# MengAiDev/SmokePhysAI

Measured on AMD Instinct MI355X. Metric: simulated+encoded frames/sec at 256^2 grid, batch 64, higher is better.
Workload: dtype f32 stencil + bf16x3 encoder (split-bf16 MFMA, fp32 accumulate)

## Files before the change

smokephysai_amd/csrc/encoder.h:

```cpp
#pragma once
#include <mutex>
#include <vector>

#include "common.h"

namespace smk {

struct EncoderDev {
    float *w1;
    float *s1, *t1;
    float *w2t;
    float *s2, *t2;
    unsigned short *w1p;
    signed char *w2i;
    float *sw2;
    int *wsum;
    unsigned short *w2q;
    unsigned short *w2s;
};

struct EncoderSkip {
    std::mutex mu;
    float *table[3][3][2] = {};
    int *ws = nullptr;
    size_t ws_tiles = 0;
    std::vector<void *> retired;
    int64_t last_total = 0;
    const int *last_count = nullptr;
    void release();
};
hipError_t encoder_skip_stats(EncoderSkip &sk, int64_t *tiles_total, int64_t *tiles_run, hipStream_t st);

hipError_t launch_fold_weights(const smk_encoder_weights &w, const EncoderDev &e, hipStream_t st);
hipError_t launch_conv1_only(const float *frames, int64_t fstride, int B, int H, int W, const EncoderDev &e, float *act,
                             hipStream_t st);
hipError_t launch_encoder_f32(const float *frames, int64_t fstride, int B, int H, int W, const EncoderDev &e,
                              float *features, hipStream_t st);

hipError_t launch_encoder_bf16(const float *frames, int64_t fstride, int B, int H, int W, const EncoderDev &e,
                               float *features, bool x3, bool tokens, hipStream_t st, EncoderSkip *skip = nullptr);
hipError_t launch_encoder_b16(const float *frames, int64_t fstride, int B, int H, int W, const EncoderDev &e,
                              float *features, bool tokens, hipStream_t st, EncoderSkip *skip = nullptr);

hipError_t launch_encoder_i8(const float *frames, int64_t fstride, int B, int H, int W, const EncoderDev &e,
                             float *features, bool tokens, hipStream_t st, EncoderSkip *skip = nullptr);

size_t conv2_train_workspace_bytes();
hipError_t launch_conv2_train_dgrad(const float *dz, const float *weight, int B, int H, int W, float *dx, void *workspace, hipStream_t st);
size_t conv1_wgrad_workspace_bytes();
hipError_t launch_conv1_train_forward(const float *x, const float *weight, const float *bias, int B, int H, int W, float *z1, hipStream_t st);
hipError_t launch_conv1_train_wgrad(const float *dz, const float *x, int B, int H, int W, float *dw, float *db, void *workspace, hipStream_t st);
size_t conv2_wgrad_workspace_bytes(int nstreams);
int conv2_wgrad_streams();
hipError_t launch_conv2_train_wgrad(const float *dz, const float *a1, int B, int H, int W, float *dw, float *db, void *workspace, hipStream_t st);
hipError_t launch_conv2_train_forward(const float *a1, const float *weight, const float *bias, int B, int H, int W, float *z2, void *workspace,
                                      hipStream_t st);

}
```

smokephysai_amd/csrc/encoder.hip:

```cpp
#include "encoder.h"

#include <stdlib.h>

namespace smk {

typedef float f32x16 __attribute__((ext_vector_type(16)));

constexpr int ENC_TH = 8, ENC_TW = 32;
constexpr int ENC_AH = ENC_TH + 2, ENC_AW = ENC_TW + 2;
constexpr int ENC_XH = ENC_TH + 8, ENC_XW = ENC_TW + 8;
constexpr int ENC_ACS = ENC_AH * ENC_AW;

__global__ void k_fold_weights(smk_encoder_weights w, EncoderDev e) {
    int t = blockIdx.x * blockDim.x + threadIdx.x;
    if (t < 64) {
        float s = w.bn1_w[t] / sqrtf(w.bn1_var[t] + 1e-5f);
        e.s1[t] = s;
        e.t1[t] = (w.conv1_b[t] - w.bn1_mean[t]) * s + w.bn1_b[t];
    }
    if (t < 128) {
        float s = w.bn2_w[t] / sqrtf(w.bn2_var[t] + 1e-5f);
        e.s2[t] = s;
        e.t2[t] = (w.conv2_b[t] - w.bn2_mean[t]) * s + w.bn2_b[t];
    }
    if (t < 64 * 49) e.w1[t] = w.conv1_w[t];
    if (t < 9 * 64 * 128) {
        int o = t % 128, c = (t / 128) % 64, tap = t / (128 * 64);
        e.w2t[t] = w.conv2_w[((size_t)o * 64 + c) * 9 + tap];
    }
    __bf16 *w1p = reinterpret_cast<__bf16 *>(e.w1p), *w2q = reinterpret_cast<__bf16 *>(e.w2q);
    if (t < 64 * 64) {
        int c = t / 64, k = t % 64, ki = k >> 3, kj = k & 7;
        float v = (ki < 7 && kj < 7) ? w.conv1_w[c * 49 + ki * 7 + kj] : 0.f;
        __bf16 hi = (__bf16)v;
        w1p[t] = hi;
        w1p[64 * 64 + t] = (__bf16)(v - (float)hi);
    }
    if (t < 36 * 128 * 16) {
        int cc = t % 16, o = (t / 16) % 128, ks = t / (16 * 128);
        int tap = ks >> 2, c = (ks & 3) * 16 + cc;
        float v = w.conv2_w[((size_t)o * 64 + c) * 9 + tap];
        __bf16 hi = (__bf16)v;
        w2q[((size_t)(ks * 2 + 0) * 128 + o) * 16 + cc] = hi;
        w2q[((size_t)(ks * 2 + 1) * 128 + o) * 16 + cc] = (__bf16)(v - (float)hi);
        __bf16 *w2s = reinterpret_cast<__bf16 *>(e.w2s);
        const int ks2 = tap * 2 + (c >> 5), c32 = c & 31;
        w2s[((size_t)(ks2 * 2 + 0) * 128 + o) * 32 + c32] = hi;
        w2s[((size_t)(ks2 * 2 + 1) * 128 + o) * 32 + c32] = (__bf16)(v - (float)hi);
    }
}

__global__ __launch_bounds__(256) void k_quant_w2(smk_encoder_weights w, EncoderDev e) {
    __shared__ float red[256];
    __shared__ int sh_h, sh_l;
    const int o = blockIdx.x, tid = threadIdx.x;
    if (tid == 0) { sh_h = 0; sh_l = 0; }
    float m = 0.f;
    for (int k = tid; k < 576; k += 256) m = fmaxf(m, fabsf(w.conv2_w[(size_t)o * 576 + k]));
    red[tid] = m;
    __syncthreads();
    for (int sft = 128; sft > 0; sft >>= 1) {
        if (tid < sft) red[tid] = fmaxf(red[tid], red[tid + sft]);
        __syncthreads();
    }
    const float wmax = red[0];
    const float sw = wmax > 0.f ? wmax / 32512.0f : 1.0f;
    if (tid == 0) e.sw2[o] = sw;
    int sum_h = 0, sum_l = 0;
    for (int k = tid; k < 576; k += 256) {
        const int c = k / 9, tap = k - 9 * c;
        const int q = (int)rintf(w.conv2_w[(size_t)o * 576 + k] / sw);
        const int h = (q + 128) >> 8, l = q - (h << 8);
        const int ks = tap * 2 + (c >> 5), cc = c & 31;
        e.w2i[((size_t)(ks * 2 + 0) * 128 + o) * 32 + cc] = (signed char)h;
        e.w2i[((size_t)(ks * 2 + 1) * 128 + o) * 32 + cc] = (signed char)l;
        sum_h += h; sum_l += l;
    }
    atomicAdd(&sh_h, sum_h);
    atomicAdd(&sh_l, sum_l);
    __syncthreads();
    if (tid == 0) { e.wsum[o] = 128 * sh_h; e.wsum[128 + o] = 128 * sh_l; }
}

hipError_t launch_fold_weights(const smk_encoder_weights &w, const EncoderDev &e, hipStream_t st) {
    hipLaunchKernelGGL(k_quant_w2, dim3(128), dim3(256), 0, st, w, e);
    int n = 9 * 64 * 128;
    hipLaunchKernelGGL(k_fold_weights, dim3((n + 255) / 256), dim3(256), 0, st, w, e);
    return hipGetLastError();
}

template <int NC>
__device__ __forceinline__ void conv1_pixel(const float (&patch)[49], const float *__restrict__ w1,
                                            const float *__restrict__ s1, const float *__restrict__ t1, int c0,
                                            float (&out)[NC]) {
#pragma unroll
    for (int cc = 0; cc < NC; ++cc) {
        const float *wc = w1 + (c0 + cc) * 49;
        float acc = 0.f;
#pragma unroll
        for (int t = 0; t < 49; ++t) acc = fmaf(patch[t], wc[t], acc);
        float y = fmaf(acc, s1[c0 + cc], t1[c0 + cc]);
        out[cc] = y > 0.f ? y : 0.f;
    }
}

__global__ __launch_bounds__(256) void k_conv1_only(const float *frames, int64_t fstride, int H, int W, EncoderDev e, float *act) {
    int b = blockIdx.z;
    int j = blockIdx.x * 64 + threadIdx.x, i = blockIdx.y * 4 + threadIdx.y;
    if (i >= H || j >= W) return;
    const float *x = frames + (size_t)b * fstride;
    float patch[49];
#pragma unroll
    for (int ki = 0; ki < 7; ++ki)
#pragma unroll
        for (int kj = 0; kj < 7; ++kj) {
            int ii = i + ki - 3, jj = j + kj - 3;
            patch[ki * 7 + kj] = (ii >= 0 && ii < H && jj >= 0 && jj < W) ? x[(size_t)ii * W + jj] : 0.f;
        }
#pragma unroll 1
    for (int c0 = 0; c0 < 64; c0 += 4) {
        float o[4];
        conv1_pixel<4>(patch, e.w1, e.s1, e.t1, c0, o);
#pragma unroll
        for (int cc = 0; cc < 4; ++cc) act[(((size_t)b * 64 + c0 + cc) * H + i) * W + j] = o[cc];
    }
}

hipError_t launch_conv1_only(const float *frames, int64_t fstride, int B, int H, int W, const EncoderDev &e, float *act,
                             hipStream_t st) {
    dim3 grid(cdiv(W, 64), cdiv(H, 4), B), block(64, 4);
    hipLaunchKernelGGL(k_conv1_only, grid, block, 0, st, frames, fstride, H, W, e, act);
    return hipGetLastError();
}

constexpr int LDS_XS = ENC_XH * ENC_XW;
constexpr int LDS_A1 = 64 * ENC_ACS;
constexpr int LDS_W2 = 64 * 128;
constexpr int LDS_F32_TOTAL = LDS_XS + LDS_A1 + 2 * LDS_W2;
constexpr int A2_PITCH = 129;

template <int PS>
__global__ __launch_bounds__(512) void k_encoder_f32(const float *__restrict__ frames, int64_t fstride, int H, int W,
                                                     EncoderDev e, float *__restrict__ features) {
    extern __shared__ __attribute__((aligned(16))) float lds[];
    float *xs = lds, *a1s = lds + LDS_XS, *w2s = lds + LDS_XS + LDS_A1;
    const int tid = threadIdx.x, lane = tid & 63;
    const int wave = __builtin_amdgcn_readfirstlane(tid >> 6);
    const int b = blockIdx.z, r0 = blockIdx.y * ENC_TH, c0 = blockIdx.x * ENC_TW;
    const float *x = frames + (size_t)b * fstride;

    for (int k = tid; k < LDS_XS; k += 512) {
        int ii = r0 - 4 + k / ENC_XW, jj = c0 - 4 + k % ENC_XW;
        xs[k] = (ii >= 0 && ii < H && jj >= 0 && jj < W) ? x[(size_t)ii * W + jj] : 0.f;
    }
    float4 wreg[4];
    {
        const float4 *src = reinterpret_cast<const float4 *>(e.w2t);
#pragma unroll
        for (int q = 0; q < 4; ++q) wreg[q] = src[q * 512 + tid];
    }
    __syncthreads();

    for (int task = wave; task < 48; task += 8) {
        const int chunk = task % 6, cq = task / 6;
        const int pix = chunk * 64 + lane;
        if (pix < ENC_ACS) {
            const int ar = pix / ENC_AW, ac = pix % ENC_AW;
            const int ii = r0 - 1 + ar, jj = c0 - 1 + ac;
            float o[8];
            if (ii >= 0 && ii < H && jj >= 0 && jj < W) {
                float patch[49];
#pragma unroll
                for (int ki = 0; ki < 7; ++ki)
#pragma unroll
                    for (int kj = 0; kj < 7; ++kj) patch[ki * 7 + kj] = xs[(ar + ki) * ENC_XW + ac + kj];
                conv1_pixel<8>(patch, e.w1, e.s1, e.t1, cq * 8, o);
            } else {
#pragma unroll
                for (int cc = 0; cc < 8; ++cc) o[cc] = 0.f;
            }
#pragma unroll
            for (int cc = 0; cc < 8; ++cc) a1s[(cq * 8 + cc) * ENC_ACS + pix] = o[cc];
        }
    }
    {
        float4 *dst = reinterpret_cast<float4 *>(w2s);
#pragma unroll
        for (int q = 0; q < 4; ++q) dst[q * 512 + tid] = wreg[q];
    }
    __syncthreads();

    f32x16 acc[4];
#pragma unroll
    for (int n = 0; n < 4; ++n)
#pragma unroll
        for (int r = 0; r < 16; ++r) acc[n][r] = 0.f;
    const int l31 = lane & 31, hi = lane >> 5;
    for (int tap = 0; tap < 9; ++tap) {
        if (tap + 1 < 9) {
            const float4 *src = reinterpret_cast<const float4 *>(e.w2t + (size_t)(tap + 1) * LDS_W2);
#pragma unroll
            for (int q = 0; q < 4; ++q) wreg[q] = src[q * 512 + tid];
        }
        const int ki = tap / 3, kj = tap % 3;
        const float *ap = a1s + hi * ENC_ACS + (wave + ki) * ENC_AW + l31 + kj;
        const float *bp = w2s + (tap & 1) * LDS_W2 + hi * 128 + l31;
#pragma unroll 4
        for (int cp = 0; cp < 32; ++cp) {
            float a = ap[cp * 2 * ENC_ACS];
#pragma unroll
            for (int n = 0; n < 4; ++n) {
                float bv = bp[cp * 2 * 128 + n * 32];
                acc[n] = __builtin_amdgcn_mfma_f32_32x32x2f32(a, bv, acc[n], 0, 0, 0);
            }
        }
        if (tap + 1 < 9) {
            float4 *dst = reinterpret_cast<float4 *>(w2s + ((tap + 1) & 1) * LDS_W2);
#pragma unroll
            for (int q = 0; q < 4; ++q) dst[q * 512 + tid] = wreg[q];
        }
        __syncthreads();
    }

    float *a2s = lds;
#pragma unroll
    for (int n = 0; n < 4; ++n) {
        const int o = n * 32 + l31;
        const float s = e.s2[o], t = e.t2[o];
#pragma unroll
        for (int r = 0; r < 16; ++r) {
            const int col = (r & 3) + 8 * (r >> 2) + 4 * hi;
            float y = fmaf(acc[n][r], s, t);
            a2s[(wave * ENC_TW + col) * A2_PITCH + o] = y > 0.f ? y : 0.f;
        }
    }
    __syncthreads();
    constexpr int CELLS_R = ENC_TH / PS, CELLS_C = ENC_TW / PS;
    const int OW = 32, OHW = 32 * 32;
    for (int k = tid; k < CELLS_R * CELLS_C * 128; k += 512) {
        const int o = k & 127, cell = k >> 7, cr = cell / CELLS_C, cc = cell % CELLS_C;
        float sum = 0.f;
        for (int rr = 0; rr < PS; ++rr)
            for (int q = 0; q < PS; ++q) sum += a2s[((cr * PS + rr) * ENC_TW + cc * PS + q) * A2_PITCH + o];
        const int pi = r0 / PS + cr, pj = c0 / PS + cc;
        features[((size_t)b * 128 + o) * OHW + pi * OW + pj] = sum * (1.0f / (PS * PS));
    }
}

hipError_t launch_encoder_f32(const float *frames, int64_t fstride, int B, int H, int W, const EncoderDev &e,
                              float *features, hipStream_t st) {
    const int PS = H / 32;
    dim3 grid(W / ENC_TW, H / ENC_TH, B), block(512);
    size_t lds_bytes = sizeof(float) * (size_t)(LDS_F32_TOTAL > 256 * A2_PITCH ? LDS_F32_TOTAL : 256 * A2_PITCH);
    once_per_device((const void *)k_encoder_f32<8>, [&] {
        (void)hipFuncSetAttribute((const void *)k_encoder_f32<2>, hipFuncAttributeMaxDynamicSharedMemorySize, (int)lds_bytes);
        (void)hipFuncSetAttribute((const void *)k_encoder_f32<4>, hipFuncAttributeMaxDynamicSharedMemorySize, (int)lds_bytes);
        (void)hipFuncSetAttribute((const void *)k_encoder_f32<8>, hipFuncAttributeMaxDynamicSharedMemorySize, (int)lds_bytes);
    });
    switch (PS) {
        case 2: hipLaunchKernelGGL(k_encoder_f32<2>, grid, block, lds_bytes, st, frames, fstride, H, W, e, features); break;
        case 4: hipLaunchKernelGGL(k_encoder_f32<4>, grid, block, lds_bytes, st, frames, fstride, H, W, e, features); break;
        case 8: hipLaunchKernelGGL(k_encoder_f32<8>, grid, block, lds_bytes, st, frames, fstride, H, W, e, features); break;
        default: return hipErrorInvalidValue;
    }
    return hipGetLastError();
}

typedef __bf16 bf16x8 __attribute__((ext_vector_type(8)));
typedef __bf16 bf16x4 __attribute__((ext_vector_type(4)));

constexpr int B3_TH = 8, B3_TW = 16;
constexpr int B3_AW = B3_TW + 2, B3_APIX = (B3_TH + 2) * B3_AW;
constexpr int B3_XH = B3_TH + 9, B3_XW = B3_TW + 9;
constexpr int B3_XS_BYTES = ((B3_XH * B3_XW * 4 + 15) / 16) * 16;
constexpr int B3_A1_PITCH = 144;
constexpr int B3_A1_ROW = B3_AW * B3_A1_PITCH + 32;
constexpr int B3_A1_BYTES = (B3_TH + 2) * B3_A1_ROW;
template <bool X3> constexpr int b3_lds_bytes() { return B3_XS_BYTES + (X3 ? 2 : 1) * B3_A1_BYTES; }

__device__ __forceinline__ void split_bf16(float v, __bf16 &hi, __bf16 &lo) {
    hi = (__bf16)v;
    lo = (__bf16)(v - (float)hi);
}

template <bool X3>
__device__ __forceinline__ void mma3(f32x16 &acc, const bf16x8 &ah, const bf16x8 &al, const bf16x8 &bh, const bf16x8 &bl) {
    if (X3) {
        acc = __builtin_amdgcn_mfma_f32_32x32x16_bf16(al, bh, acc, 0, 0, 0);
        acc = __builtin_amdgcn_mfma_f32_32x32x16_bf16(ah, bl, acc, 0, 0, 0);
    }
    acc = __builtin_amdgcn_mfma_f32_32x32x16_bf16(ah, bh, acc, 0, 0, 0);
}

__device__ __forceinline__ float bn_relu(float a, float s, float t) {
    float y = fmaf(a, s, t);
    return y > 0.f ? y : 0.f;
}

constexpr int B3_W1_PITCH = 144;
constexpr int B3_W1_BYTES = 64 * B3_W1_PITCH;
constexpr int B3_ST_BYTES = 2 * 64 * 4;
template <bool X3> constexpr int b3_lds_total() { return b3_lds_bytes<X3>() + (X3 ? 2 : 1) * B3_W1_BYTES + B3_ST_BYTES; }

__device__ __forceinline__ int tiles_to_run(const int *__restrict__ list, const int *__restrict__ count, int ntiles) {
    return list ? __builtin_amdgcn_readfirstlane(*count) : ntiles;
}
__device__ __forceinline__ int tile_at(const int *__restrict__ list, int k) {
    return list ? __builtin_amdgcn_readfirstlane(list[k]) : k;
}

template <bool X3, int PS, bool TOKENS>
__global__ __launch_bounds__(256, 2) void k_encoder_bf16(const float *__restrict__ frames, int64_t fstride, int H, int W,
                                                      EncoderDev e, float *__restrict__ features, int lg_tiles_x,
                                                      int lg_tiles_per_frame, int ntiles, int stagger,
                                                      const int *__restrict__ list, const int *__restrict__ count) {
    extern __shared__ __attribute__((aligned(16))) unsigned char smem[];
    float *xs = reinterpret_cast<float *>(smem);
    unsigned char *a1h = smem + B3_XS_BYTES, *a1l = a1h + B3_A1_BYTES;
    unsigned char *w1s = a1h + (X3 ? 2 : 1) * B3_A1_BYTES;
    float *st1 = reinterpret_cast<float *>(w1s + (X3 ? 2 : 1) * B3_W1_BYTES);
    const int tid = threadIdx.x, lane = tid & 63, r = lane & 31, hi = lane >> 5;
    const int wave = __builtin_amdgcn_readfirstlane(tid >> 6);

    if (tid < 128) st1[tid] = tid < 64 ? e.s1[tid] : e.t1[tid - 64];
    {
        constexpr int NCH = (X3 ? 2 : 1) * 64 * 8;
        const uint4 *src = reinterpret_cast<const uint4 *>(e.w1p);
        for (int c = tid; c < NCH; c += 256) {
            const int row = c >> 3, u = c & 7;
            *reinterpret_cast<uint4 *>(w1s + row * B3_W1_PITCH + u * 16) = src[c];
        }
    }
    const int o = wave * 32 + r;
    const float s2 = e.s2[o], t2 = e.t2[o];
    const int lane_b = (o * 2 + hi) * 16;
    const __amdgpu_buffer_rsrc_t wrsrc =
        __builtin_amdgcn_make_buffer_rsrc(const_cast<unsigned short *>(e.w2q), 0, 36 * 2 * 4096, 0x00020000);
    typedef unsigned int u32x4 __attribute__((ext_vector_type(4)));
    auto load_b = [&](int kn, int part) -> uint4 {
        const u32x4 v = __builtin_amdgcn_raw_buffer_load_b128(wrsrc, lane_b, (kn * 2 + part) * 4096, 0);
        return make_uint4(v[0], v[1], v[2], v[3]);
    };
    constexpr int RING = 6;
    uint4 bqh[RING], bql[RING];
#pragma unroll
    for (int k = 0; k < RING - 1; ++k) {
        bqh[k] = load_b(k, 0);
        if (X3) bql[k] = load_b(k, 1);
    }
    const int lane_off = (r >> 4) * 4 * B3_A1_ROW + (r & 15) * B3_A1_PITCH + 8 * hi * 2;

    auto x_fetch = [&](int t, int k) -> float {
        if (k >= B3_XH * B3_XW) return 0.f;
        const int bb = t >> lg_tiles_per_frame, rem = t & ((1 << lg_tiles_per_frame) - 1);
        const int rr0 = (rem >> lg_tiles_x) * B3_TH, cc0 = (rem & ((1 << lg_tiles_x) - 1)) * B3_TW;
        const int row = k / B3_XW, col = k - row * B3_XW;
        const int ii = rr0 - 4 + row, jj = cc0 - 4 + col;
        const bool ok = row < B3_XH - 1 && col < B3_XW - 1 && ii >= 0 && ii < H && jj >= 0 && jj < W;
        return ok ? frames[(size_t)bb * fstride + (size_t)ii * W + jj] : 0.f;
    };
    int k = blockIdx.x;
    const int nrun = tiles_to_run(list, count, ntiles);
    if (nrun == ntiles) list = nullptr;
    int t = k < nrun ? tile_at(list, k) : 0;
    if (stagger > 0 && ((blockIdx.x / 256) & 1))
        for (int i = 0; i < stagger; ++i) __builtin_amdgcn_s_sleep(127);
    if (k < nrun) {
        xs[tid] = x_fetch(t, tid);
        if (tid + 256 < B3_XH * B3_XW) xs[tid + 256] = x_fetch(t, tid + 256);
    }
    __syncthreads();

    for (; k < nrun; k += gridDim.x) {
        const int b = t >> lg_tiles_per_frame, rem = t & ((1 << lg_tiles_per_frame) - 1);
        const int r0 = (rem >> lg_tiles_x) * B3_TH, c0 = (rem & ((1 << lg_tiles_x) - 1)) * B3_TW;

        __builtin_amdgcn_s_setprio(0);
        auto x_frags = [&](int pb, bf16x8 (&xh)[4], bf16x8 (&xl)[4], int &aoff, bool &valid, bool &inimg) {
            const int pix = pb * 32 + r;
            valid = pix < B3_APIX;
            const int pc = valid ? pix : B3_APIX - 1;
            const int ar = pc / B3_AW, ac = pc - ar * B3_AW;
            const int ii = r0 - 1 + ar, jj = c0 - 1 + ac;
            inimg = valid && ii >= 0 && ii < H && jj >= 0 && jj < W;
            aoff = ar * B3_A1_ROW + ac * B3_A1_PITCH;
            const float *xp = xs + (ar + hi) * B3_XW + ac;
#pragma unroll
            for (int s = 0; s < 4; ++s)
#pragma unroll
                for (int j = 0; j < 8; ++j) {
                    __bf16 vh, vl;
                    split_bf16(xp[s * 2 * B3_XW + j], vh, vl);
                    xh[s][j] = vh; xl[s][j] = vl;
                }
        };
        auto conv1_store = [&](const f32x16 &acc, int cb, int aoff, bool valid, bool inimg) {
#pragma unroll
            for (int q = 0; q < 4; ++q) {
                const int ch0 = cb * 32 + 8 * q + 4 * hi;
                const float4 sc = *reinterpret_cast<const float4 *>(st1 + ch0);
                const float4 sh = *reinterpret_cast<const float4 *>(st1 + 64 + ch0);
                const float scv[4] = {sc.x, sc.y, sc.z, sc.w}, shv[4] = {sh.x, sh.y, sh.z, sh.w};
                bf16x4 vh, vl;
#pragma unroll
                for (int i = 0; i < 4; ++i) {
                    const float y = inimg ? bn_relu(acc[4 * q + i], scv[i], shv[i]) : 0.f;
                    __bf16 a, bb;
                    split_bf16(y, a, bb);
                    vh[i] = a; vl[i] = bb;
                }
                if (valid) {
                    *reinterpret_cast<bf16x4 *>(a1h + aoff + ch0 * 2) = vh;
                    if (X3) *reinterpret_cast<bf16x4 *>(a1l + aoff + ch0 * 2) = vl;
                }
            }
        };
        {
            bf16x8 xh[4], xl[4];
            int aoff; bool valid, inimg;
            x_frags(wave, xh, xl, aoff, valid, inimg);
            f32x16 acc0, acc1;
#pragma unroll
            for (int g = 0; g < 16; ++g) { acc0[g] = 0.f; acc1[g] = 0.f; }
            const unsigned char *wrow = w1s + r * B3_W1_PITCH + 8 * hi * 2;
#pragma unroll
            for (int s = 0; s < 4; ++s) {
                const bf16x8 a0h = *reinterpret_cast<const bf16x8 *>(wrow + s * 32);
                const bf16x8 a1hh = *reinterpret_cast<const bf16x8 *>(wrow + 32 * B3_W1_PITCH + s * 32);
                const bf16x8 a0l = X3 ? *reinterpret_cast<const bf16x8 *>(wrow + B3_W1_BYTES + s * 32) : a0h;
                const bf16x8 a1l_ = X3 ? *reinterpret_cast<const bf16x8 *>(wrow + B3_W1_BYTES + 32 * B3_W1_PITCH + s * 32) : a1hh;
                mma3<X3>(acc0, a0h, a0l, xh[s], xl[s]);
                mma3<X3>(acc1, a1hh, a1l_, xh[s], xl[s]);
            }
            conv1_store(acc0, 0, aoff, valid, inimg);
            conv1_store(acc1, 1, aoff, valid, inimg);
        }
        {
            bf16x8 xh[4], xl[4];
            int aoff; bool valid, inimg;
            const int cb = wave & 1;
            x_frags(4 + (wave >> 1), xh, xl, aoff, valid, inimg);
            f32x16 acc;
#pragma unroll
            for (int g = 0; g < 16; ++g) acc[g] = 0.f;
            const unsigned char *wrow = w1s + (cb * 32 + r) * B3_W1_PITCH + 8 * hi * 2;
#pragma unroll
            for (int s = 0; s < 4; ++s) {
                const bf16x8 ah = *reinterpret_cast<const bf16x8 *>(wrow + s * 32);
                const bf16x8 al = X3 ? *reinterpret_cast<const bf16x8 *>(wrow + B3_W1_BYTES + s * 32) : ah;
                mma3<X3>(acc, ah, al, xh[s], xl[s]);
            }
            conv1_store(acc, cb, aoff, valid, inimg);
        }
        __syncthreads();
        __builtin_amdgcn_s_setprio(1);

        const int kn = k + gridDim.x;
        const int tn = kn < nrun ? tile_at(list, kn) : 0;
        float xr0 = 0.f, xr1 = 0.f;
        if (kn < nrun) {
            xr0 = x_fetch(tn, tid);
            xr1 = x_fetch(tn, tid + 256);
        }

        f32x16 acc[4];
#pragma unroll
        for (int mi = 0; mi < 4; ++mi)
#pragma unroll
            for (int g = 0; g < 16; ++g) acc[mi][g] = 0.f;
        auto load_a = [&](int k, bf16x8 (&ah)[4], bf16x8 (&al)[4]) {
            const int tap = k >> 2, ks = k & 3, ki = tap / 3, kj = tap - 3 * ki;
            const int abase = lane_off + ki * B3_A1_ROW + kj * B3_A1_PITCH + ks * 32;
#pragma unroll
            for (int mi = 0; mi < 4; ++mi) {
                ah[mi] = *reinterpret_cast<const bf16x8 *>(a1h + abase + mi * B3_A1_ROW);
                if (X3) al[mi] = *reinterpret_cast<const bf16x8 *>(a1l + abase + mi * B3_A1_ROW);
            }
        };
        bf16x8 ahA[4], alA[4], ahB[4], alB[4];
        load_a(0, ahA, alA);
        constexpr int UNR = 6;
#pragma unroll 1
        for (int k0 = 0; k0 < 36; k0 += UNR) {
#pragma unroll
            for (int u = 0; u < UNR; ++u) {
                const int k = k0 + u;
                {
                    int kn = k + RING - 1;
                    kn = kn >= 36 ? kn - 36 : kn;
                    kn = __builtin_amdgcn_readfirstlane(kn);
                    bqh[(u + RING - 1) % RING] = load_b(kn, 0);
                    if (X3) bql[(u + RING - 1) % RING] = load_b(kn, 1);
                }
                if (k + 1 < 36) {
                    if (u & 1) load_a(k + 1, ahA, alA); else load_a(k + 1, ahB, alB);
                }
                const bf16x8 bh = __builtin_bit_cast(bf16x8, bqh[u % RING]);
                const bf16x8 bl = X3 ? __builtin_bit_cast(bf16x8, bql[u % RING]) : bh;
#pragma unroll
                for (int mi = 0; mi < 4; ++mi) {
                    if (u & 1) mma3<X3>(acc[mi], ahB[mi], alB[mi], bh, bl); else mma3<X3>(acc[mi], ahA[mi], alA[mi], bh, bl);
                }
                constexpr int NMF = X3 ? 12 : 4, NDS = X3 ? 8 : 4, NVM = X3 ? 2 : 1;
#pragma unroll
                for (int i = 0; i < NMF; ++i) {
                    __builtin_amdgcn_sched_group_barrier(0x008, 1, 0);
                    if (i < NDS) __builtin_amdgcn_sched_group_barrier(0x100, 1, 0);
                    else if (i < NDS + NVM) __builtin_amdgcn_sched_group_barrier(0x020, 1, 0);
                }
                __builtin_amdgcn_sched_barrier(0);
            }
        }

        auto out_index = [&](int pi, int pj) -> size_t {
            return TOKENS ? ((size_t)b * 1024 + pi * 32 + pj) * 128 + o : ((size_t)b * 128 + o) * 1024 + pi * 32 + pj;
        };
        if (PS == 2) {
#pragma unroll
            for (int mp = 0; mp < 2; ++mp)
#pragma unroll
                for (int qr = 0; qr < 2; ++qr)
#pragma unroll
                    for (int qc = 0; qc < 2; ++qc)
#pragma unroll
                        for (int cg = 0; cg < 2; ++cg) {
                            float sum = 0.f;
#pragma unroll
                            for (int mi = 2 * mp; mi < 2 * mp + 2; ++mi)
#pragma unroll
                                for (int i = 2 * cg; i < 2 * cg + 2; ++i) sum += bn_relu(acc[mi][4 * (2 * qr + qc) + i], s2, t2);
                            features[out_index((r0 + 2 * mp + 4 * qr) / 2, (c0 + 8 * qc + 4 * hi + 2 * cg) / 2)] = sum * 0.25f;
                        }
        } else if (PS == 4) {
#pragma unroll
            for (int qr = 0; qr < 2; ++qr)
#pragma unroll
                for (int qc = 0; qc < 2; ++qc) {
                    float sum = 0.f;
#pragma unroll
                    for (int mi = 0; mi < 4; ++mi)
#pragma unroll
                        for (int i = 0; i < 4; ++i) sum += bn_relu(acc[mi][4 * (2 * qr + qc) + i], s2, t2);
                    features[out_index((r0 + 4 * qr) / 4, (c0 + 8 * qc + 4 * hi) / 4)] = sum * (1.0f / 16);
                }
        } else {
            float cell[2];
#pragma unroll
            for (int qc = 0; qc < 2; ++qc) {
                float sum = 0.f;
#pragma unroll
                for (int mi = 0; mi < 4; ++mi)
#pragma unroll
                    for (int qr = 0; qr < 2; ++qr)
#pragma unroll
                        for (int i = 0; i < 4; ++i) sum += bn_relu(acc[mi][4 * (2 * qr + qc) + i], s2, t2);
                cell[qc] = sum;
            }
            const float other0 = __shfl_xor(cell[0], 32), other1 = __shfl_xor(cell[1], 32);
            const float total = hi == 0 ? cell[0] + other0 : cell[1] + other1;
            features[out_index(r0 / 8, c0 / 8 + hi)] = total * (1.0f / 64);
        }

        xs[tid] = xr0;
        if (tid + 256 < B3_XH * B3_XW) xs[tid + 256] = xr1;
        __syncthreads();
        t = tn;
    }
}

#ifndef S16_PRIO_CONV1
#define S16_PRIO_CONV1 0
#define S16_PRIO_KLOOP 1
#endif
constexpr int S16_A1_BYTES = B3_APIX * 128;
constexpr int S16_LDS = B3_XS_BYTES + 2 * S16_A1_BYTES + 2 * B3_W1_BYTES + B3_ST_BYTES;
typedef float f32x4v __attribute__((ext_vector_type(4)));

template <int PS, bool TOKENS>
__global__ __launch_bounds__(256, 2) void k_encoder_b16(const float *__restrict__ frames, int64_t fstride, int H, int W,
                                                     EncoderDev e, float *__restrict__ features, int lg_tiles_x,
                                                     int lg_tiles_per_frame, int ntiles, int stagger,
                                                     const int *__restrict__ list, const int *__restrict__ count) {
    extern __shared__ __attribute__((aligned(16))) unsigned char smem[];
    unsigned int *xs = reinterpret_cast<unsigned int *>(smem);
    unsigned char *a1h = smem + B3_XS_BYTES, *a1l = a1h + S16_A1_BYTES;
    unsigned char *w1s = a1l + S16_A1_BYTES;
    float *st1 = reinterpret_cast<float *>(w1s + 2 * B3_W1_BYTES);
    const int tid = threadIdx.x, lane = tid & 63, r = lane & 31, hi = lane >> 5;
    const int wave = __builtin_amdgcn_readfirstlane(tid >> 6);

    if (tid < 128) st1[tid] = tid < 64 ? e.s1[tid] : e.t1[tid - 64];
    {
        const uint4 *src = reinterpret_cast<const uint4 *>(e.w1p);
        for (int c = tid; c < 2 * 64 * 8; c += 256) {
            const int row = c >> 3, u = c & 7;
            *reinterpret_cast<uint4 *>(w1s + row * B3_W1_PITCH + u * 16) = src[c];
        }
    }
    const int px = lane & 15, kg = lane >> 4;
    const int o0 = wave * 32 + px;
    const float s2a = e.s2[o0], t2a = e.t2[o0], s2b = e.s2[o0 + 16], t2b = e.t2[o0 + 16];
    const int lane_b = o0 * 64 + kg * 16;
    const __amdgpu_buffer_rsrc_t wrsrc =
        __builtin_amdgcn_make_buffer_rsrc(const_cast<unsigned short *>(e.w2s), 0, 18 * 2 * 8192, 0x00020000);
    typedef unsigned int u32x4 __attribute__((ext_vector_type(4)));
    auto load_b = [&](int ks, int part, int nt) -> uint4 {
        const u32x4 v = __builtin_amdgcn_raw_buffer_load_b128(wrsrc, lane_b, (ks * 2 + part) * 8192 + nt * 1024, 0);
        return make_uint4(v.x, v.y, v.z, v.w);
    };
    constexpr int RING = 2;
    uint4 bq[RING][2][2];
#pragma unroll
    for (int k = 0; k < RING - 1; ++k)
#pragma unroll
        for (int nt = 0; nt < 2; ++nt) {
            bq[k][nt][0] = load_b(k, 0, nt);
            bq[k][nt][1] = load_b(k, 1, nt);
        }

    auto x_fetch = [&](int t, int k) -> float {
        if (k >= B3_XH * B3_XW) return 0.f;
        const int bb = t >> lg_tiles_per_frame, rem = t & ((1 << lg_tiles_per_frame) - 1);
        const int rr0 = (rem >> lg_tiles_x) * B3_TH, cc0 = (rem & ((1 << lg_tiles_x) - 1)) * B3_TW;
        const int row = k / B3_XW, col = k - row * B3_XW;
        const int ii = rr0 - 4 + row, jj = cc0 - 4 + col;
        const bool ok = row < B3_XH - 1 && col < B3_XW - 1 && ii >= 0 && ii < H && jj >= 0 && jj < W;
        return ok ? frames[(size_t)bb * fstride + (size_t)ii * W + jj] : 0.f;
    };
    auto pack_split = [](float v) -> unsigned int {
        __bf16 vh, vl;
        split_bf16(v, vh, vl);
        return (unsigned int)__builtin_bit_cast(unsigned short, vh) | ((unsigned int)__builtin_bit_cast(unsigned short, vl) << 16);
    };
    int k = blockIdx.x;
    const int nrun = tiles_to_run(list, count, ntiles);
    if (nrun == ntiles) list = nullptr;
    int t = k < nrun ? tile_at(list, k) : 0;
    if (stagger > 0 && ((blockIdx.x / 256) & 1))
        for (int i = 0; i < stagger; ++i) __builtin_amdgcn_s_sleep(127);
    if (k < nrun) {
        xs[tid] = pack_split(x_fetch(t, tid));
        if (tid + 256 < B3_XH * B3_XW) xs[tid + 256] = pack_split(x_fetch(t, tid + 256));
    }
    __syncthreads();

    for (; k < nrun; k += gridDim.x) {
        const int b = t >> lg_tiles_per_frame, rem = t & ((1 << lg_tiles_per_frame) - 1);
        const int r0 = (rem >> lg_tiles_x) * B3_TH, c0 = (rem & ((1 << lg_tiles_x) - 1)) * B3_TW;

        __builtin_amdgcn_s_setprio(S16_PRIO_CONV1);
#ifdef SMK_ENC_ABLATE
        const bool abl_conv1 = !((SMK_ENC_ABLATE & 1) && k != (int)blockIdx.x);
#else
        constexpr bool abl_conv1 = true;
#endif
        auto x_frags = [&](int pb, bf16x8 (&xh)[4], bf16x8 (&xl)[4], int &pix, bool &valid, bool &inimg) {
            const int pp = pb * 32 + r;
            valid = pp < B3_APIX;
            pix = valid ? pp : B3_APIX - 1;
            const int ar = pix / B3_AW, ac = pix - ar * B3_AW;
            const int ii = r0 - 1 + ar, jj = c0 - 1 + ac;
            inimg = valid && ii >= 0 && ii < H && jj >= 0 && jj < W;
            const unsigned int *xp = xs + (ar + hi) * B3_XW + ac;
#pragma unroll
            for (int s = 0; s < 4; ++s) {
                unsigned int wh[4], wl[4];
#pragma unroll
                for (int jj = 0; jj < 4; ++jj) {
                    const unsigned int e0 = xp[s * 2 * B3_XW + 2 * jj], e1 = xp[s * 2 * B3_XW + 2 * jj + 1];
                    wh[jj] = __builtin_amdgcn_perm(e1, e0, 0x05040100u);
                    wl[jj] = __builtin_amdgcn_perm(e1, e0, 0x07060302u);
                }
                xh[s] = __builtin_bit_cast(bf16x8, make_uint4(wh[0], wh[1], wh[2], wh[3]));
                xl[s] = __builtin_bit_cast(bf16x8, make_uint4(wl[0], wl[1], wl[2], wl[3]));
            }
        };
        auto conv1_store = [&](const f32x16 &acc, int cb, int pix, bool valid, bool inimg) {
            const int sw = pix & 7;
#pragma unroll
            for (int q = 0; q < 4; ++q) {
                const int ch0 = cb * 32 + 8 * q + 4 * hi;
                const float4 sc = *reinterpret_cast<const float4 *>(st1 + ch0);
                const float4 sh = *reinterpret_cast<const float4 *>(st1 + 64 + ch0);
                const float scv[4] = {sc.x, sc.y, sc.z, sc.w}, shv[4] = {sh.x, sh.y, sh.z, sh.w};
                bf16x4 vh, vl;
#pragma unroll
                for (int i = 0; i < 4; ++i) {
                    const float y = inimg ? bn_relu(acc[4 * q + i], scv[i], shv[i]) : 0.f;
                    __bf16 a, bb;
                    split_bf16(y, a, bb);
                    vh[i] = a; vl[i] = bb;
                }
                if (valid) {
                    const int off = pix * 128 + (((cb * 4 + q) ^ sw) * 16) + 8 * hi;
                    *reinterpret_cast<bf16x4 *>(a1h + off) = vh;
                    *reinterpret_cast<bf16x4 *>(a1l + off) = vl;
                }
            }
        };
        if (abl_conv1) {
            bf16x8 xh[4], xl[4];
            int pix; bool valid, inimg;
            x_frags(wave, xh, xl, pix, valid, inimg);
            f32x16 acc0, acc1;
#pragma unroll
            for (int g = 0; g < 16; ++g) { acc0[g] = 0.f; acc1[g] = 0.f; }
            const unsigned char *wrow = w1s + r * B3_W1_PITCH + 8 * hi * 2;
#pragma unroll
            for (int s = 0; s < 4; ++s) {
                const bf16x8 a0h = *reinterpret_cast<const bf16x8 *>(wrow + s * 32);
                const bf16x8 a1hh = *reinterpret_cast<const bf16x8 *>(wrow + 32 * B3_W1_PITCH + s * 32);
                const bf16x8 a0l = *reinterpret_cast<const bf16x8 *>(wrow + B3_W1_BYTES + s * 32);
                const bf16x8 a1l_ = *reinterpret_cast<const bf16x8 *>(wrow + B3_W1_BYTES + 32 * B3_W1_PITCH + s * 32);
                mma3<true>(acc0, a0h, a0l, xh[s], xl[s]);
                mma3<true>(acc1, a1hh, a1l_, xh[s], xl[s]);
            }
            conv1_store(acc0, 0, pix, valid, inimg);
            conv1_store(acc1, 1, pix, valid, inimg);
        }
        if (abl_conv1) {
            bf16x8 xh[4], xl[4];
            int pix; bool valid, inimg;
            const int cb = wave & 1;
            x_frags(4 + (wave >> 1), xh, xl, pix, valid, inimg);
            f32x16 acc;
#pragma unroll
            for (int g = 0; g < 16; ++g) acc[g] = 0.f;
            const unsigned char *wrow = w1s + (cb * 32 + r) * B3_W1_PITCH + 8 * hi * 2;
#pragma unroll
            for (int s = 0; s < 4; ++s) {
                const bf16x8 ah = *reinterpret_cast<const bf16x8 *>(wrow + s * 32);
                const bf16x8 al = *reinterpret_cast<const bf16x8 *>(wrow + B3_W1_BYTES + s * 32);
                mma3<true>(acc, ah, al, xh[s], xl[s]);
            }
            conv1_store(acc, cb, pix, valid, inimg);
        }
#if !defined(SMK_ENC_ABLATE) || !(SMK_ENC_ABLATE & 4)
        __syncthreads();
#endif
        __builtin_amdgcn_s_setprio(S16_PRIO_KLOOP);

        const int kn = k + gridDim.x;
        const int tn = kn < nrun ? tile_at(list, kn) : 0;
        float xr0 = 0.f, xr1 = 0.f;
        if (kn < nrun) {
            xr0 = x_fetch(tn, tid);
            xr1 = x_fetch(tn, tid + 256);
        }

        f32x4v acc[8][2];
#pragma unroll
        for (int mt = 0; mt < 8; ++mt)
#pragma unroll
            for (int nt = 0; nt < 2; ++nt)
#pragma unroll
                for (int g = 0; g < 4; ++g) acc[mt][nt][g] = 0.f;
        const int c16[2] = {kg << 4, (4 + kg) << 4};
        auto tap_consts = [&](int ki, int kj, int (&om)[4]) {
#pragma unroll
            for (int m = 0; m < 4; ++m) om[m] = ((px + kj) << 7) ^ (((px + kj + 2 * (m + ki)) & 7) << 4);
        };
        auto load_a = [&](int ki, int half, int hm, const int (&om)[4], bf16x8 (&ah)[4], bf16x8 (&al)[4]) {
            const unsigned char *ph = a1h + ki * (B3_AW * 128), *pl = a1l + ki * (B3_AW * 128);
#pragma unroll
            for (int m = 0; m < 4; ++m) {
                const int off = om[m] ^ c16[half];
                ah[m] = *reinterpret_cast<const bf16x8 *>(ph + off + (4 * hm + m) * (B3_AW * 128));
                al[m] = *reinterpret_cast<const bf16x8 *>(pl + off + (4 * hm + m) * (B3_AW * 128));
            }
        };
        bf16x8 ahA[4], alA[4], ahB[4], alB[4];
        int om[4];
        tap_consts(0, 0, om);
        load_a(0, 0, 0, om, ahA, alA);
        int ki = 0, kj = 0;
#pragma unroll 1
        for (int tap = 0; tap < 9; ++tap) {
#pragma unroll
            for (int u = 0; u < 4; ++u) {
                const int half = u >> 1, hm = u & 1, slot = half % RING;
                if (hm == 0) {
                    int kn = tap * 2 + half + RING - 1;
                    kn = kn >= 18 ? kn - 18 : kn;
                    kn = __builtin_amdgcn_readfirstlane(kn);
#pragma unroll
                    for (int nt = 0; nt < 2; ++nt) {
                        bq[(slot + RING - 1) % RING][nt][0] = load_b(kn, 0, nt);
                        bq[(slot + RING - 1) % RING][nt][1] = load_b(kn, 1, nt);
                    }
                }
                if (u < 3) {
                    if (u & 1) load_a(ki, (u + 1) >> 1, (u + 1) & 1, om, ahA, alA);
                    else load_a(ki, (u + 1) >> 1, (u + 1) & 1, om, ahB, alB);
                } else if (tap < 8) {
                    kj = kj == 2 ? 0 : kj + 1;
                    ki = kj == 0 ? ki + 1 : ki;
                    tap_consts(ki, kj, om);
                    load_a(ki, 0, 0, om, ahA, alA);
                }
#pragma unroll
                for (int pr = 0; pr < 3; ++pr)
#pragma unroll
                    for (int m = 0; m < 4; ++m)
#pragma unroll
                        for (int nt = 0; nt < 2; ++nt) {
                            const bf16x8 bh = __builtin_bit_cast(bf16x8, bq[slot][nt][0]);
                            const bf16x8 bl = __builtin_bit_cast(bf16x8, bq[slot][nt][1]);
                            f32x4v &c = acc[4 * hm + m][nt];
                            const bf16x8 ah = (u & 1) ? ahB[m] : ahA[m], al = (u & 1) ? alB[m] : alA[m];
#if defined(SMK_ENC_ABLATE) && (SMK_ENC_ABLATE & 8)
                            asm volatile("" :: "v"(al), "v"(ah), "v"(bh), "v"(bl), "v"(c));
#else
                            if (pr == 0) c = __builtin_amdgcn_mfma_f32_16x16x32_bf16(al, bh, c, 0, 0, 0);
                            else if (pr == 1) c = __builtin_amdgcn_mfma_f32_16x16x32_bf16(ah, bl, c, 0, 0, 0);
                            else c = __builtin_amdgcn_mfma_f32_16x16x32_bf16(ah, bh, c, 0, 0, 0);
#endif
                        }
#pragma unroll
                for (int i = 0; i < 24; ++i) {
                    __builtin_amdgcn_sched_group_barrier(0x008, 1, 0);
                    if (i % 3 == 0) __builtin_amdgcn_sched_group_barrier(0x100, 1, 0);
                    else if (hm == 0 && (i == 1 || i == 2 || i == 4 || i == 5)) __builtin_amdgcn_sched_group_barrier(0x020, 1, 0);
                }
                __builtin_amdgcn_sched_barrier(0);
            }
        }

        auto out_index = [&](int pi, int pj, int o) -> size_t {
            return TOKENS ? ((size_t)b * 1024 + pi * 32 + pj) * 128 + o : ((size_t)b * 128 + o) * 1024 + pi * 32 + pj;
        };
#if defined(SMK_ENC_ABLATE) && (SMK_ENC_ABLATE & 2)
#pragma unroll
        for (int mt = 0; mt < 8; ++mt) asm volatile("" :: "v"(acc[mt][0]), "v"(acc[mt][1]));
        if (false)
#endif
#pragma unroll
        for (int nt = 0; nt < 2; ++nt) {
            const float s2 = nt ? s2b : s2a, t2 = nt ? t2b : t2a;
            const int o = o0 + 16 * nt;
            if (PS == 2) {
#pragma unroll
                for (int mp = 0; mp < 4; ++mp)
#pragma unroll
                    for (int cg = 0; cg < 2; ++cg) {
                        float sum = 0.f;
#pragma unroll
                        for (int mt = 2 * mp; mt < 2 * mp + 2; ++mt)
#pragma unroll
                            for (int i = 2 * cg; i < 2 * cg + 2; ++i) sum += bn_relu(acc[mt][nt][i], s2, t2);
                        features[out_index((r0 + 2 * mp) / 2, (c0 + 4 * kg + 2 * cg) / 2, o)] = sum * 0.25f;
                    }
            } else if (PS == 4) {
#pragma unroll
                for (int mq = 0; mq < 2; ++mq) {
                    float sum = 0.f;
#pragma unroll
                    for (int mt = 4 * mq; mt < 4 * mq + 4; ++mt)
#pragma unroll
                        for (int i = 0; i < 4; ++i) sum += bn_relu(acc[mt][nt][i], s2, t2);
                    features[out_index((r0 + 4 * mq) / 4, (c0 + 4 * kg) / 4, o)] = sum * (1.0f / 16);
                }
            } else {
                float sum = 0.f;
#pragma unroll
                for (int mt = 0; mt < 8; ++mt)
#pragma unroll
                    for (int i = 0; i < 4; ++i) sum += bn_relu(acc[mt][nt][i], s2, t2);
                const float other = __shfl_xor(sum, 16);
                const float total = (kg & 1) == 0 ? sum + other : other + sum;
                if ((kg & 1) == 0) features[out_index(r0 / 8, c0 / 8 + (kg >> 1), o)] = total * (1.0f / 64);
            }
        }

        xs[tid] = pack_split(xr0);
        if (tid + 256 < B3_XH * B3_XW) xs[tid + 256] = pack_split(xr1);
#if !defined(SMK_ENC_ABLATE) || !(SMK_ENC_ABLATE & 4)
        __syncthreads();
#endif
        t = tn;
    }
}

constexpr int C1_WP = 52;
__global__ __launch_bounds__(256) void k_conv1_train_fwd(const float *__restrict__ x, int H, int W, const float *__restrict__ w,
                                                        const float *__restrict__ bias, float *__restrict__ z1) {
    __shared__ __attribute__((aligned(16))) float ws[64 * C1_WP];
    __shared__ float xs[10][264];
    const int tid = threadIdx.x, b = blockIdx.z, i0 = blockIdx.y * 4, j0 = blockIdx.x * 256;
    for (int k = tid; k < 64 * C1_WP; k += 256) {
        const int c = k / C1_WP, t = k - c * C1_WP;
        ws[k] = t < 49 ? w[c * 49 + t] : 0.f;
    }
    const float *xb = x + (size_t)b * H * W;
    for (int k = tid; k < 10 * 262; k += 256) {
        const int r = k / 262, cc = k - r * 262, ii = i0 - 3 + r, jj = j0 - 3 + cc;
        const int ci = ii < 0 ? 0 : (ii > H - 1 ? H - 1 : ii), cj = jj < 0 ? 0 : (jj > W - 1 ? W - 1 : jj);
        const float v = xb[(size_t)ci * W + cj];
        xs[r][cc] = (ii == ci && jj == cj) ? v : 0.f;
    }
    __syncthreads();
    const int jq = tid & 63, row = tid >> 6;
    float win[7][10];
#pragma unroll
    for (int r = 0; r < 7; ++r)
#pragma unroll
        for (int cc = 0; cc < 10; ++cc) win[r][cc] = xs[row + r][4 * jq + cc];
    const int i = i0 + row, j = j0 + 4 * jq;
    if (i >= H || j >= W) return;
    float *dst = z1 + ((size_t)b * 64 * H + i) * W + j;
#pragma unroll 1
    for (int c = 0; c < 64; ++c) {
        float wv[C1_WP];
#pragma unroll
        for (int q = 0; q < C1_WP / 4; ++q) {
            const float4 t4 = *reinterpret_cast<const float4 *>(&ws[c * C1_WP + 4 * q]);
            wv[4 * q] = t4.x; wv[4 * q + 1] = t4.y; wv[4 * q + 2] = t4.z; wv[4 * q + 3] = t4.w;
        }
        float acc[4] = {0.f, 0.f, 0.f, 0.f};
#pragma unroll
        for (int ki = 0; ki < 7; ++ki)
#pragma unroll
            for (int kj = 0; kj < 7; ++kj)
#pragma unroll
                for (int p = 0; p < 4; ++p) acc[p] = fmaf(win[ki][kj + p], wv[ki * 7 + kj], acc[p]);
        const float bb = bias ? bias[c] : 0.f;
        *reinterpret_cast<float4 *>(dst + (size_t)c * H * W) = make_float4(acc[0] + bb, acc[1] + bb, acc[2] + bb, acc[3] + bb);
    }
}

constexpr int C1G_PX = 4 * 64;
constexpr int C1G_ZP = C1G_PX * 4 + 4;
__global__ __launch_bounds__(256) void k_conv1_train_wgrad(const float *__restrict__ dz, const float *__restrict__ x, int H, int W, int tiles_x,
                                                          int tiles_per_frame, int ntiles, float *__restrict__ part) {
    extern __shared__ __attribute__((aligned(16))) float smemf[];
    float *zs = smemf;
    float *xs = smemf + 16 * C1G_ZP;
    const int tid = threadIdx.x;
    const int st = tid / 112, rem = tid - st * 112, cg = rem / 7, ky = rem - cg * 7;
    float acc[4][7], dbs[4] = {0.f, 0.f, 0.f, 0.f};
#pragma unroll
    for (int c = 0; c < 4; ++c)
#pragma unroll
        for (int k = 0; k < 7; ++k) acc[c][k] = 0.f;
    const size_t plane = (size_t)H * W;
    for (int t = blockIdx.x; t < ntiles; t += gridDim.x) {
        const int b = t / tiles_per_frame, rm = t - b * tiles_per_frame;
        const int i0 = (rm / tiles_x) * 4, j0 = (rm % tiles_x) * 64;
#pragma unroll 4
        for (int k = 0; k < 16; ++k) {
            const int it = tid + 256 * k, g = it >> 8, p = it & 255, r = p >> 6, cc = p & 63;
            const float *src = dz + ((size_t)b * 64 + 4 * g) * plane + (size_t)(i0 + r) * W + j0 + cc;
            *reinterpret_cast<float4 *>(&zs[g * C1G_ZP + 4 * p]) = make_float4(src[0], src[plane], src[2 * plane], src[3 * plane]);
        }
        const float *xb = x + (size_t)b * plane;
        for (int k = tid; k < 10 * 70; k += 256) {
            const int r = k / 70, cc = k - r * 70, ii = i0 - 3 + r, jj = j0 - 3 + cc;
            const int ci = ii < 0 ? 0 : (ii > H - 1 ? H - 1 : ii), cj = jj < 0 ? 0 : (jj > W - 1 ? W - 1 : jj);
            const float v = xb[(size_t)ci * W + cj];
            xs[r * 72 + cc] = (ii == ci && jj == cj) ? v : 0.f;
        }
        __syncthreads();
        if (tid < 224) {
#pragma unroll 1
            for (int r = 2 * st; r < 2 * st + 2; ++r) {
                const float *xr = xs + (r + ky) * 72;
                float xv[7];
#pragma unroll
                for (int k = 0; k < 6; ++k) xv[k + 1] = xr[k];
#pragma unroll 4
                for (int cc = 0; cc < 64; ++cc) {
#pragma unroll
                    for (int k = 0; k < 6; ++k) xv[k] = xv[k + 1];
                    xv[6] = xr[cc + 6];
                    const float4 d = *reinterpret_cast<const float4 *>(&zs[cg * C1G_ZP + 4 * (r * 64 + cc)]);
                    const float dv[4] = {d.x, d.y, d.z, d.w};
#pragma unroll
                    for (int c = 0; c < 4; ++c) {
#pragma unroll
                        for (int k = 0; k < 7; ++k) acc[c][k] = fmaf(dv[c], xv[k], acc[c][k]);
                        if (ky == 0) dbs[c] += dv[c];
                    }
                }
            }
        }
        __syncthreads();
    }
    float *ex = smemf;
    if (st == 1 && tid < 224) {
#pragma unroll
        for (int c = 0; c < 4; ++c) {
#pragma unroll
            for (int k = 0; k < 7; ++k) ex[rem * 32 + c * 7 + k] = acc[c][k];
            ex[rem * 32 + 28 + c] = dbs[c];
        }
    }
    __syncthreads();
    if (st == 0) {
        float *dst = part + (size_t)blockIdx.x * (64 * 49 + 64);
#pragma unroll
        for (int c = 0; c < 4; ++c) {
#pragma unroll
            for (int k = 0; k < 7; ++k) dst[(4 * cg + c) * 49 + ky * 7 + k] = acc[c][k] + ex[rem * 32 + c * 7 + k];
            if (ky == 0) dst[64 * 49 + 4 * cg + c] = dbs[c] + ex[rem * 32 + 28 + c];
        }
    }
}

__global__ __launch_bounds__(256) void k_conv1_wgrad_finish(const float *__restrict__ part, int nparts, float *__restrict__ dw, float *__restrict__ db) {
    const int i = blockIdx.x * 256 + threadIdx.x;
    if (i >= 64 * 49 + 64) return;
    float s = 0.f;
    for (int k = 0; k < nparts; ++k) s += part[(size_t)k * (64 * 49 + 64) + i];
    if (i < 64 * 49) dw[i] = s;
    else if (db) db[i - 64 * 49] = s;
}

constexpr int C1G_LDS = (16 * C1G_ZP + 10 * 72) * 4;
int conv1_wgrad_parts() { return device_num_cu() * 2; }
size_t conv1_wgrad_workspace_bytes() { return (size_t)conv1_wgrad_parts() * (64 * 49 + 64) * sizeof(float); }

hipError_t launch_conv1_train_forward(const float *x, const float *weight, const float *bias, int B, int H, int W, float *z1, hipStream_t st) {
    if (W % 4 != 0 || B < 1) return hipErrorInvalidValue;
    hipLaunchKernelGGL(k_conv1_train_fwd, dim3(cdiv(W, 256), cdiv(H, 4), B), dim3(256), 0, st, x, H, W, weight, bias, z1);
    return hipGetLastError();
}

hipError_t launch_conv1_train_wgrad(const float *dz, const float *x, int B, int H, int W, float *dw, float *db, void *workspace, hipStream_t st) {
    if (H % 4 != 0 || W % 64 != 0 || B < 1) return hipErrorInvalidValue;
    const int tiles_x = W / 64, tiles_per_frame = tiles_x * (H / 4), ntiles = B * tiles_per_frame;
    int nparts = conv1_wgrad_parts();
    once_per_device((const void *)k_conv1_train_wgrad, [&] {
        (void)hipFuncSetAttribute((const void *)k_conv1_train_wgrad, hipFuncAttributeMaxDynamicSharedMemorySize, C1G_LDS);
    });
    const int grid = nparts < ntiles ? nparts : ntiles;
    float *part = static_cast<float *>(workspace);
    hipLaunchKernelGGL(k_conv1_train_wgrad, dim3(grid), dim3(256), C1G_LDS, st, dz, x, H, W, tiles_x, tiles_per_frame, ntiles, part);
    hipLaunchKernelGGL(k_conv1_wgrad_finish, dim3(cdiv(64 * 49 + 64, 256)), dim3(256), 0, st, part, grid, dw, db);
    return hipGetLastError();
}

constexpr int C2F_LDS = 3 * S16_A1_BYTES;
__device__ __forceinline__ void split3_bf16(float v, __bf16 &h, __bf16 &m, __bf16 &l) {
    h = (__bf16)v;
    const float r1 = v - (float)h;
    m = (__bf16)r1;
    l = (__bf16)(r1 - (float)m);
}

__global__ __launch_bounds__(256, 2) void k_conv2_fwd_b16(const float *__restrict__ a1, int H, int W, const unsigned short *__restrict__ w2s,
                                                       const float *__restrict__ bias, float *__restrict__ z2, int tiles_x,
                                                       int tiles_per_frame, int ntiles) {
    extern __shared__ __attribute__((aligned(16))) unsigned char smem[];
    unsigned char *a1p[3] = {smem, smem + S16_A1_BYTES, smem + 2 * S16_A1_BYTES};
    const int tid = threadIdx.x, lane = tid & 63;
    const int wave = __builtin_amdgcn_readfirstlane(tid >> 6);
    const int px = lane & 15, kg = lane >> 4;
    const int o0 = wave * 32 + px;
    const float b2a = bias ? bias[o0] : 0.f, b2b = bias ? bias[o0 + 16] : 0.f;
    const int lane_b = o0 * 64 + kg * 16;
    const __amdgpu_buffer_rsrc_t wrsrc =
        __builtin_amdgcn_make_buffer_rsrc(const_cast<unsigned short *>(w2s), 0, 18 * 3 * 8192, 0x00020000);
    typedef unsigned int u32x4 __attribute__((ext_vector_type(4)));
    auto load_b = [&](int ks, int part, int nt) -> uint4 {
        const u32x4 v = __builtin_amdgcn_raw_buffer_load_b128(wrsrc, lane_b, (ks * 3 + part) * 8192 + nt * 1024, 0);
        return make_uint4(v.x, v.y, v.z, v.w);
    };
    uint4 bq[2][2][3];
#pragma unroll
    for (int nt = 0; nt < 2; ++nt)
#pragma unroll
        for (int part = 0; part < 3; ++part) bq[0][nt][part] = load_b(0, part, nt);
    const size_t plane = (size_t)H * W;
    constexpr int ITEMS = (B3_TH + 2) * 8 * B3_AW;
    constexpr int NIT = (ITEMS + 255) / 256;

    for (int t = blockIdx.x; t < ntiles; t += gridDim.x) {
        const int b = t / tiles_per_frame, rem = t - b * tiles_per_frame;
        const int r0 = (rem / tiles_x) * B3_TH, c0 = (rem % tiles_x) * B3_TW;
        __builtin_amdgcn_s_setprio(S16_PRIO_CONV1);
        {
            const float *ab = a1 + (size_t)b * 64 * plane;
            float v[NIT][8];
#pragma unroll
            for (int j = 0; j < NIT; ++j) {
                int idx = tid + 256 * j;
                idx = idx < ITEMS ? idx : ITEMS - 1;
                const int row = idx / (8 * B3_AW), rm = idx - row * (8 * B3_AW), g = rm / B3_AW, pc = rm - g * B3_AW;
                const int ii = r0 - 1 + row, jj = c0 - 1 + pc;
                const int ci = ii < 0 ? 0 : (ii > H - 1 ? H - 1 : ii), cj = jj < 0 ? 0 : (jj > W - 1 ? W - 1 : jj);
                const float *src = ab + (size_t)(8 * g) * plane + (size_t)ci * W + cj;
#pragma unroll
                for (int c = 0; c < 8; ++c) v[j][c] = src[(size_t)c * plane];
            }
#pragma unroll
            for (int j = 0; j < NIT; ++j) {
                const int idx = tid + 256 * j;
                if (idx < ITEMS) {
                    const int row = idx / (8 * B3_AW), rm = idx - row * (8 * B3_AW), g = rm / B3_AW, pc = rm - g * B3_AW;
                    const int ii = r0 - 1 + row, jj = c0 - 1 + pc;
                    const bool in = ii >= 0 && ii < H && jj >= 0 && jj < W;
                    const int p = row * B3_AW + pc;
                    bf16x8 vh, vm, vl;
#pragma unroll
                    for (int c = 0; c < 8; ++c) {
                        __bf16 hh, mm, ll;
                        split3_bf16(in ? v[j][c] : 0.f, hh, mm, ll);
                        vh[c] = hh; vm[c] = mm; vl[c] = ll;
                    }
                    const int off = p * 128 + ((g ^ (p & 7)) * 16);
                    *reinterpret_cast<bf16x8 *>(a1p[0] + off) = vh;
                    *reinterpret_cast<bf16x8 *>(a1p[1] + off) = vm;
                    *reinterpret_cast<bf16x8 *>(a1p[2] + off) = vl;
                }
            }
        }
        __syncthreads();
        __builtin_amdgcn_s_setprio(S16_PRIO_KLOOP);

        f32x4v acc[8][2];
#pragma unroll
        for (int mt = 0; mt < 8; ++mt)
#pragma unroll
            for (int nt = 0; nt < 2; ++nt)
#pragma unroll
                for (int g = 0; g < 4; ++g) acc[mt][nt][g] = 0.f;
        const int c16[2] = {kg << 4, (4 + kg) << 4};
        auto tap_consts8 = [&](int ki, int kj, int (&om8)[8]) {
#pragma unroll
            for (int m = 0; m < 8; ++m) om8[m] = ((px + kj) << 7) ^ (((px + kj + 2 * (m + ki)) & 7) << 4);
        };
        auto load_a = [&](int ki, int half, int mq, const int (&om8)[8], bf16x8 (&af)[3][2]) {
#pragma unroll
            for (int j = 0; j < 2; ++j) {
                const int m = 2 * mq + j;
                const int off = (om8[m] ^ c16[half]) + (ki + m) * (B3_AW * 128);
#pragma unroll
                for (int part = 0; part < 3; ++part) af[part][j] = *reinterpret_cast<const bf16x8 *>(a1p[part] + off);
            }
        };
        bf16x8 afA[3][2], afB[3][2];
        int om8[8];
        tap_consts8(0, 0, om8);
        load_a(0, 0, 0, om8, afA);
        int ki = 0, kj = 0;
#pragma unroll 1
        for (int tap = 0; tap < 9; ++tap) {
#pragma unroll
            for (int u = 0; u < 8; ++u) {
                const int half = u >> 2, mq = u & 3, slot = half;
                if (mq == 0) {
                    int kn = tap * 2 + half + 1;
                    kn = kn >= 18 ? kn - 18 : kn;
                    kn = __builtin_amdgcn_readfirstlane(kn);
#pragma unroll
                    for (int nt = 0; nt < 2; ++nt)
#pragma unroll
                        for (int part = 0; part < 3; ++part) bq[slot ^ 1][nt][part] = load_b(kn, part, nt);
                }
                if (u < 7) {
                    if (u & 1) load_a(ki, (u + 1) >> 2, (u + 1) & 3, om8, afA);
                    else load_a(ki, (u + 1) >> 2, (u + 1) & 3, om8, afB);
                } else if (tap < 8) {
                    kj = kj == 2 ? 0 : kj + 1;
                    ki = kj == 0 ? ki + 1 : ki;
                    tap_consts8(ki, kj, om8);
                    load_a(ki, 0, 0, om8, afA);
                }
#pragma unroll
                for (int pr = 0; pr < 6; ++pr)
#pragma unroll
                    for (int j = 0; j < 2; ++j)
#pragma unroll
                        for (int nt = 0; nt < 2; ++nt) {
                            constexpr int PA[6] = {2, 0, 1, 1, 0, 0}, PB[6] = {0, 2, 1, 0, 1, 0};
                            const bf16x8 av = (u & 1) ? afB[PA[pr]][j] : afA[PA[pr]][j];
                            const bf16x8 bv = __builtin_bit_cast(bf16x8, bq[slot][nt][PB[pr]]);
                            f32x4v &c = acc[2 * mq + j][nt];
                            c = __builtin_amdgcn_mfma_f32_16x16x32_bf16(av, bv, c, 0, 0, 0);
                        }
#pragma unroll
                for (int i = 0; i < 24; ++i) {
                    __builtin_amdgcn_sched_group_barrier(0x008, 1, 0);
                    if (i % 4 == 0) __builtin_amdgcn_sched_group_barrier(0x100, 1, 0);
                    else if (mq == 0 && i < 9) __builtin_amdgcn_sched_group_barrier(0x020, 1, 0);
                }
                __builtin_amdgcn_sched_barrier(0);
            }
        }

#pragma unroll
        for (int nt = 0; nt < 2; ++nt) {
            const float bb = nt ? b2b : b2a;
            float *dst = z2 + ((size_t)b * 128 + o0 + 16 * nt) * plane + (size_t)r0 * W + c0 + 4 * kg;
#pragma unroll
            for (int mt = 0; mt < 8; ++mt) {
                const f32x4v c = acc[mt][nt];
                *reinterpret_cast<float4 *>(dst + (size_t)mt * W) = make_float4(c[0] + bb, c[1] + bb, c[2] + bb, c[3] + bb);
            }
        }
        __syncthreads();
    }
}

__global__ __launch_bounds__(256, 2) void k_conv2_dgrad_b16(const float *__restrict__ dz, int H, int W, const unsigned short *__restrict__ w2d,
                                                         float *__restrict__ dx, int tiles_x, int tiles_per_frame, int ntiles) {
    extern __shared__ __attribute__((aligned(16))) unsigned char smem[];
    unsigned char *a1h = smem, *a1l = a1h + S16_A1_BYTES;
    const int tid = threadIdx.x, lane = tid & 63;
    const int wave = __builtin_amdgcn_readfirstlane(tid >> 6);
    const int px = lane & 15, kg = lane >> 4;
    const int mh = wave & 1, nh = wave >> 1;
    const int c0o = nh * 32 + px;
    const int lane_b = c0o * 64 + kg * 16;
    const __amdgpu_buffer_rsrc_t wrsrc =
        __builtin_amdgcn_make_buffer_rsrc(const_cast<unsigned short *>(w2d), 0, 2 * 18 * 2 * 4096, 0x00020000);
    typedef unsigned int u32x4 __attribute__((ext_vector_type(4)));
    auto load_b = [&](int ks36, int part, int nt) -> uint4 {
        const u32x4 v = __builtin_amdgcn_raw_buffer_load_b128(wrsrc, lane_b, (ks36 * 2 + part) * 4096 + nt * 1024, 0);
        return make_uint4(v.x, v.y, v.z, v.w);
    };
    uint4 bq[2][2][2];
#pragma unroll
    for (int nt = 0; nt < 2; ++nt) {
        bq[0][nt][0] = load_b(0, 0, nt);
        bq[0][nt][1] = load_b(0, 1, nt);
    }
    const size_t plane = (size_t)H * W;
    constexpr int ITEMS = (B3_TH + 2) * 8 * B3_AW, NIT = (ITEMS + 255) / 256;
    const unsigned char *a1h_w = a1h + mh * 4 * (B3_AW * 128), *a1l_w = a1l + mh * 4 * (B3_AW * 128);
    const int c16[2] = {kg << 4, (4 + kg) << 4};

    for (int t = blockIdx.x; t < ntiles; t += gridDim.x) {
        const int b = t / tiles_per_frame, rem = t - b * tiles_per_frame;
        const int r0 = (rem / tiles_x) * B3_TH, c0 = (rem % tiles_x) * B3_TW;
        f32x4v acc[4][2];
#pragma unroll
        for (int m = 0; m < 4; ++m)
#pragma unroll
            for (int nt = 0; nt < 2; ++nt)
#pragma unroll
                for (int g = 0; g < 4; ++g) acc[m][nt][g] = 0.f;
#pragma unroll 1
        for (int pass = 0; pass < 2; ++pass) {
            __builtin_amdgcn_s_setprio(S16_PRIO_CONV1);
            {
                const float *ab = dz + ((size_t)b * 128 + 64 * pass) * plane;
                float v[NIT][8];
#pragma unroll
                for (int j = 0; j < NIT; ++j) {
                    int idx = tid + 256 * j;
                    idx = idx < ITEMS ? idx : ITEMS - 1;
                    const int row = idx / (8 * B3_AW), rm = idx - row * (8 * B3_AW), g = rm / B3_AW, pc = rm - g * B3_AW;
                    const int ii = r0 - 1 + row, jj = c0 - 1 + pc;
                    const int ci = ii < 0 ? 0 : (ii > H - 1 ? H - 1 : ii), cj = jj < 0 ? 0 : (jj > W - 1 ? W - 1 : jj);
                    const float *src = ab + (size_t)(8 * g) * plane + (size_t)ci * W + cj;
#pragma unroll
                    for (int c = 0; c < 8; ++c) v[j][c] = src[(size_t)c * plane];
                }
#pragma unroll
                for (int j = 0; j < NIT; ++j) {
                    const int idx = tid + 256 * j;
                    if (idx < ITEMS) {
                        const int row = idx / (8 * B3_AW), rm = idx - row * (8 * B3_AW), g = rm / B3_AW, pc = rm - g * B3_AW;
                        const int ii = r0 - 1 + row, jj = c0 - 1 + pc;
                        const bool in = ii >= 0 && ii < H && jj >= 0 && jj < W;
                        const int p = row * B3_AW + pc;
                        bf16x8 vh, vl;
#pragma unroll
                        for (int c = 0; c < 8; ++c) {
                            __bf16 hh, ll;
                            split_bf16(in ? v[j][c] : 0.f, hh, ll);
                            vh[c] = hh; vl[c] = ll;
                        }
                        const int off = p * 128 + ((g ^ (p & 7)) * 16);
                        *reinterpret_cast<bf16x8 *>(a1h + off) = vh;
                        *reinterpret_cast<bf16x8 *>(a1l + off) = vl;
                    }
                }
            }
            __syncthreads();
            __builtin_amdgcn_s_setprio(S16_PRIO_KLOOP);
            auto tap_consts = [&](int ki, int kj, int (&om)[4]) {
#pragma unroll
                for (int m = 0; m < 4; ++m) om[m] = ((px + kj) << 7) ^ (((px + kj + 2 * (m + ki)) & 7) << 4);
            };
            auto load_a = [&](int ki, int half, const int (&om)[4], bf16x8 (&ah)[4], bf16x8 (&al)[4]) {
                const unsigned char *ph = a1h_w + ki * (B3_AW * 128), *pl = a1l_w + ki * (B3_AW * 128);
#pragma unroll
                for (int m = 0; m < 4; ++m) {
                    const int off = om[m] ^ c16[half];
                    ah[m] = *reinterpret_cast<const bf16x8 *>(ph + off + m * (B3_AW * 128));
                    al[m] = *reinterpret_cast<const bf16x8 *>(pl + off + m * (B3_AW * 128));
                }
            };
            bf16x8 ahA[4], alA[4], ahB[4], alB[4];
            int om[4];
            tap_consts(0, 0, om);
            load_a(0, 0, om, ahA, alA);
            int ki = 0, kj = 0;
#pragma unroll 1
            for (int tap = 0; tap < 9; ++tap) {
#pragma unroll
                for (int half = 0; half < 2; ++half) {
                    const int slot = half;
                    {
                        int kn = pass * 18 + tap * 2 + half + 1;
                        kn = kn >= 36 ? kn - 36 : kn;
                        kn = __builtin_amdgcn_readfirstlane(kn);
#pragma unroll
                        for (int nt = 0; nt < 2; ++nt) {
                            bq[slot ^ 1][nt][0] = load_b(kn, 0, nt);
                            bq[slot ^ 1][nt][1] = load_b(kn, 1, nt);
                        }
                    }
                    if (half == 0) {
                        load_a(ki, 1, om, ahB, alB);
                    } else if (tap < 8) {
                        kj = kj == 2 ? 0 : kj + 1;
                        ki = kj == 0 ? ki + 1 : ki;
                        tap_consts(ki, kj, om);
                        load_a(ki, 0, om, ahA, alA);
                    }
#pragma unroll
                    for (int pr = 0; pr < 3; ++pr)
#pragma unroll
                        for (int m = 0; m < 4; ++m)
#pragma unroll
                            for (int nt = 0; nt < 2; ++nt) {
                                const bf16x8 bh = __builtin_bit_cast(bf16x8, bq[slot][nt][0]);
                                const bf16x8 bl = __builtin_bit_cast(bf16x8, bq[slot][nt][1]);
                                f32x4v &c = acc[m][nt];
                                const bf16x8 ah = half ? ahB[m] : ahA[m], al = half ? alB[m] : alA[m];
                                if (pr == 0) c = __builtin_amdgcn_mfma_f32_16x16x32_bf16(al, bh, c, 0, 0, 0);
                                else if (pr == 1) c = __builtin_amdgcn_mfma_f32_16x16x32_bf16(ah, bl, c, 0, 0, 0);
                                else c = __builtin_amdgcn_mfma_f32_16x16x32_bf16(ah, bh, c, 0, 0, 0);
                            }
#pragma unroll
                    for (int i = 0; i < 24; ++i) {
                        __builtin_amdgcn_sched_group_barrier(0x008, 1, 0);
                        if (i % 3 == 0) __builtin_amdgcn_sched_group_barrier(0x100, 1, 0);
                        else if (i == 1 || i == 2 || i == 4 || i == 5) __builtin_amdgcn_sched_group_barrier(0x020, 1, 0);
                    }
                    __builtin_amdgcn_sched_barrier(0);
                }
            }
            __syncthreads();
        }
#pragma unroll
        for (int nt = 0; nt < 2; ++nt) {
            float *dst = dx + ((size_t)b * 64 + c0o + 16 * nt) * plane + (size_t)(r0 + 4 * mh) * W + c0 + 4 * kg;
#pragma unroll
            for (int m = 0; m < 4; ++m) {
                const f32x4v c = acc[m][nt];
                *reinterpret_cast<float4 *>(dst + (size_t)m * W) = make_float4(c[0], c[1], c[2], c[3]);
            }
        }
    }
}

__global__ void k_split_conv2_weights_dgrad(const float *__restrict__ w, unsigned short *__restrict__ w2d_) {
    const int t = blockIdx.x * blockDim.x + threadIdx.x;
    if (t >= 9 * 64 * 128) return;
    const int o = t % 128, c = (t / 128) % 64, tap = t / (64 * 128);
    const float v = w[((size_t)o * 64 + c) * 9 + tap];
    const int ky = tap / 3, kx = tap - 3 * ky, tapf = (2 - ky) * 3 + (2 - kx);
    __bf16 *w2d = reinterpret_cast<__bf16 *>(w2d_);
    const __bf16 hi = (__bf16)v;
    const int pass = o >> 6, ol = o & 63, ks = tapf * 2 + (ol >> 5), o32 = ol & 31;
    const size_t base = ((size_t)(pass * 18 + ks) * 2) * 64 * 32;
    w2d[base + (size_t)c * 32 + o32] = hi;
    w2d[base + (size_t)64 * 32 + (size_t)c * 32 + o32] = (__bf16)(v - (float)hi);
}

hipError_t launch_conv2_train_dgrad(const float *dz, const float *weight, int B, int H, int W, float *dx, void *workspace, hipStream_t st) {
    if (H % B3_TH != 0 || W % B3_TW != 0 || B < 1) return hipErrorInvalidValue;
    unsigned short *w2d = static_cast<unsigned short *>(workspace);
    hipLaunchKernelGGL(k_split_conv2_weights_dgrad, dim3(cdiv(9 * 64 * 128, 256)), dim3(256), 0, st, weight, w2d);
    const int tiles_x = W / B3_TW, tiles_per_frame = tiles_x * (H / B3_TH), ntiles = B * tiles_per_frame;
    constexpr int lds = 2 * S16_A1_BYTES;
    const int wgs_per_cu = device_cached_int((const void *)k_conv2_dgrad_b16, [] {
        (void)hipFuncSetAttribute((const void *)k_conv2_dgrad_b16, hipFuncAttributeMaxDynamicSharedMemorySize, lds);
        int n = 0;
        if (hipOccupancyMaxActiveBlocksPerMultiprocessor(&n, (const void *)k_conv2_dgrad_b16, 256, lds) != hipSuccess || n < 1) n = 2;
        return n;
    });
    int nwg = device_num_cu() * wgs_per_cu;
    if (nwg > ntiles) nwg = ntiles;
    hipLaunchKernelGGL(k_conv2_dgrad_b16, dim3(nwg), dim3(256), lds, st, dz, H, W, w2d, dx, tiles_x, tiles_per_frame, ntiles);
    return hipGetLastError();
}

constexpr int WG_OG = 32;
constexpr int WG_ZP = 272;
constexpr int WG_AC = 336;
constexpr int WG_Z_BYTES = WG_OG * WG_ZP;
constexpr int WG_A_BYTES = 64 * WG_AC;
constexpr int WG_H_BYTES = 64 * 10 * 2 * 2;
constexpr int WG_LDS = 2 * (WG_Z_BYTES + WG_A_BYTES + WG_H_BYTES);

__global__ __launch_bounds__(256, 2) void k_conv2_wgrad_b16(const float *__restrict__ dz, const float *__restrict__ a1, int H, int W, int tiles_x,
                                                         int tiles_per_frame, int ntiles, int nstreams, float *__restrict__ part,
                                                         float *__restrict__ dbpart) {
    extern __shared__ __attribute__((aligned(16))) unsigned char smem[];
    unsigned char *zh = smem, *zl = zh + WG_Z_BYTES, *ah = zl + WG_Z_BYTES, *al = ah + WG_A_BYTES, *hh = al + WG_A_BYTES, *hl = hh + WG_H_BYTES;
    const int tid = threadIdx.x, lane = tid & 63;
    const int wave = __builtin_amdgcn_readfirstlane(tid >> 6);
    const int n15 = lane & 15, kg = lane >> 4;
    const int xcd = blockIdx.x & 7, og = (blockIdx.x >> 3) & 3, stream = (blockIdx.x >> 5) * 8 + xcd;
    const size_t plane = (size_t)H * W;
    f32x4v acc[2][9];
#pragma unroll
    for (int m = 0; m < 2; ++m)
#pragma unroll
        for (int t9 = 0; t9 < 9; ++t9)
#pragma unroll
            for (int g = 0; g < 4; ++g) acc[m][t9][g] = 0.f;
    float dbsum = 0.f;

    for (int t = stream; t < ntiles; t += nstreams) {
        const int b = t / tiles_per_frame, rem = t - b * tiles_per_frame;
        const int r0 = (rem / tiles_x) * B3_TH, c0 = (rem % tiles_x) * B3_TW;
        {
            const int o = tid >> 3, row = tid & 7;
            const float *src = dz + ((size_t)b * 128 + og * WG_OG + o) * plane + (size_t)(r0 + row) * W + c0;
            float4 v[4];
#pragma unroll
            for (int q = 0; q < 4; ++q) v[q] = *reinterpret_cast<const float4 *>(src + 4 * q);
#pragma unroll
            for (int hlf = 0; hlf < 2; ++hlf) {
                const float f[8] = {v[2 * hlf].x, v[2 * hlf].y, v[2 * hlf].z, v[2 * hlf].w, v[2 * hlf + 1].x, v[2 * hlf + 1].y, v[2 * hlf + 1].z, v[2 * hlf + 1].w};
                bf16x8 vh, vl;
#pragma unroll
                for (int c = 0; c < 8; ++c) {
                    __bf16 a_, b_;
                    split_bf16(f[c], a_, b_);
                    vh[c] = a_; vl[c] = b_;
                    dbsum += f[c];
                }
                const int off = o * WG_ZP + (row * 16 + 8 * hlf) * 2;
                *reinterpret_cast<bf16x8 *>(zh + off) = vh;
                *reinterpret_cast<bf16x8 *>(zl + off) = vl;
            }
        }
#pragma unroll
        for (int j = 0; j < 3; ++j) {
            const int it = tid + 256 * j;
            if (it < 640) {
                const int c = it / 10, row = it - c * 10;
                const int ii = r0 - 1 + row;
                const bool rin = ii >= 0 && ii < H;
                const float *src = a1 + ((size_t)b * 64 + c) * plane + (size_t)(rin ? ii : 0) * W + c0;
                float4 v[4];
#pragma unroll
                for (int q = 0; q < 4; ++q) v[q] = *reinterpret_cast<const float4 *>(src + 4 * q);
                const float lft = (rin && c0 > 0) ? src[-1] : 0.f, rgt = (rin && c0 + 16 < W) ? src[16] : 0.f;
#pragma unroll
                for (int hlf = 0; hlf < 2; ++hlf) {
                    const float f[8] = {v[2 * hlf].x, v[2 * hlf].y, v[2 * hlf].z, v[2 * hlf].w, v[2 * hlf + 1].x, v[2 * hlf + 1].y, v[2 * hlf + 1].z, v[2 * hlf + 1].w};
                    bf16x8 vh, vl;
#pragma unroll
                    for (int e = 0; e < 8; ++e) {
                        __bf16 a_, b_;
                        split_bf16(rin ? f[e] : 0.f, a_, b_);
                        vh[e] = a_; vl[e] = b_;
                    }
                    const int off = c * WG_AC + row * 32 + 16 * hlf;
                    *reinterpret_cast<bf16x8 *>(ah + off) = vh;
                    *reinterpret_cast<bf16x8 *>(al + off) = vl;
                }
                __bf16 lh_, ll_, rh_, rl_;
                split_bf16(lft, lh_, ll_);
                split_bf16(rgt, rh_, rl_);
                __bf16 *ph = reinterpret_cast<__bf16 *>(hh) + (c * 10 + row) * 2, *pl = reinterpret_cast<__bf16 *>(hl) + (c * 10 + row) * 2;
                ph[0] = lh_; ph[1] = rh_;
                pl[0] = ll_; pl[1] = rl_;
            }
        }
        __syncthreads();
        const int cw = wave * 16 + n15;
        const int x0 = 8 * (kg & 1);
#pragma unroll
        for (int s4 = 0; s4 < 4; ++s4) {
            const int prow = 2 * s4 + (kg >> 1);
            bf16x8 azh[2], azl[2];
#pragma unroll
            for (int m = 0; m < 2; ++m) {
                const int off = (m * 16 + n15) * WG_ZP + (prow * 16 + x0) * 2;
                azh[m] = *reinterpret_cast<const bf16x8 *>(zh + off);
                azl[m] = *reinterpret_cast<const bf16x8 *>(zl + off);
            }
#pragma unroll
            for (int ky = 0; ky < 3; ++ky) {
                const int arow = prow + ky;
                const int rbase = cw * WG_AC + arow * 32;
                typedef unsigned int u32x4 __attribute__((ext_vector_type(4)));
                const u32x4 ch = *reinterpret_cast<const u32x4 *>(ah + rbase + 2 * x0), cl = *reinterpret_cast<const u32x4 *>(al + rbase + 2 * x0);
                const int lo_off = x0 ? rbase + 14 : -1, ro_off = x0 ? -1 : rbase + 16;
                const int hidx = ((cw * 10 + arow) * 2) * 2;
                const unsigned int leh = lo_off >= 0 ? *reinterpret_cast<const unsigned short *>(ah + lo_off) : *reinterpret_cast<const unsigned short *>(hh + hidx);
                const unsigned int lel = lo_off >= 0 ? *reinterpret_cast<const unsigned short *>(al + lo_off) : *reinterpret_cast<const unsigned short *>(hl + hidx);
                const unsigned int reh = ro_off >= 0 ? *reinterpret_cast<const unsigned short *>(ah + ro_off) : *reinterpret_cast<const unsigned short *>(hh + hidx + 2);
                const unsigned int rel = ro_off >= 0 ? *reinterpret_cast<const unsigned short *>(al + ro_off) : *reinterpret_cast<const unsigned short *>(hl + hidx + 2);
#pragma unroll
                for (int kx = 0; kx < 3; ++kx) {
                    u32x4 fh, fl;
                    if (kx == 1) {
                        fh = ch; fl = cl;
                    } else if (kx == 0) {
                        fh[0] = leh | (ch[0] << 16); fl[0] = lel | (cl[0] << 16);
#pragma unroll
                        for (int i = 1; i < 4; ++i) {
                            fh[i] = __builtin_amdgcn_alignbit(ch[i], ch[i - 1], 16);
                            fl[i] = __builtin_amdgcn_alignbit(cl[i], cl[i - 1], 16);
                        }
                    } else {
#pragma unroll
                        for (int i = 0; i < 3; ++i) {
                            fh[i] = __builtin_amdgcn_alignbit(ch[i + 1], ch[i], 16);
                            fl[i] = __builtin_amdgcn_alignbit(cl[i + 1], cl[i], 16);
                        }
                        fh[3] = (ch[3] >> 16) | (reh << 16); fl[3] = (cl[3] >> 16) | (rel << 16);
                    }
                    const bf16x8 bh = __builtin_bit_cast(bf16x8, fh), bl = __builtin_bit_cast(bf16x8, fl);
                    const int t9 = ky * 3 + kx;
#pragma unroll
                    for (int m = 0; m < 2; ++m) {
                        f32x4v &c = acc[m][t9];
                        c = __builtin_amdgcn_mfma_f32_16x16x32_bf16(azl[m], bh, c, 0, 0, 0);
                        c = __builtin_amdgcn_mfma_f32_16x16x32_bf16(azh[m], bl, c, 0, 0, 0);
                        c = __builtin_amdgcn_mfma_f32_16x16x32_bf16(azh[m], bh, c, 0, 0, 0);
                    }
                }
            }
        }
        __syncthreads();
    }
    float *dst = part + ((size_t)stream * 4 + og) * (WG_OG * 9 * 64);
#pragma unroll
    for (int m = 0; m < 2; ++m)
#pragma unroll
        for (int t9 = 0; t9 < 9; ++t9)
#pragma unroll
            for (int g = 0; g < 4; ++g) dst[((size_t)(m * 16 + 4 * kg + g) * 9 + t9) * 64 + wave * 16 + n15] = acc[m][t9][g];
    float sdb = dbsum;
    sdb += __shfl_xor(sdb, 1); sdb += __shfl_xor(sdb, 2); sdb += __shfl_xor(sdb, 4);
    if ((tid & 7) == 0) dbpart[((size_t)stream * 4 + og) * WG_OG + (tid >> 3)] = sdb;
}

__global__ __launch_bounds__(256) void k_conv2_wgrad_finish(const float *__restrict__ part, const float *__restrict__ dbpart, int nstreams,
                                                          float *__restrict__ dw, float *__restrict__ db) {
    const int i = blockIdx.x * 256 + threadIdx.x;
    if (i < 128 * 9 * 64) {
        const int c = i & 63, t9 = (i >> 6) % 9, o = i / (9 * 64);
        const float *src = part + ((size_t)(o >> 5) * (WG_OG * 9 * 64)) + ((size_t)(o & 31) * 9 + t9) * 64 + c;
        float s = 0.f;
        for (int st = 0; st < nstreams; ++st) s += src[(size_t)st * 4 * (WG_OG * 9 * 64)];
        dw[((size_t)o * 64 + c) * 9 + t9] = s;
    }
    if (db && i < 128) {
        float s = 0.f;
        for (int st = 0; st < nstreams; ++st) s += dbpart[((size_t)st * 4 + (i >> 5)) * WG_OG + (i & 31)];
        db[i] = s;
    }
}

size_t conv2_wgrad_workspace_bytes(int nstreams) { return ((size_t)nstreams * 4 * (WG_OG * 9 * 64) + (size_t)nstreams * 4 * WG_OG) * sizeof(float); }
int conv2_wgrad_streams() { return (device_num_cu() * 2 / 32) * 8; }

hipError_t launch_conv2_train_wgrad(const float *dz, const float *a1, int B, int H, int W, float *dw, float *db, void *workspace, hipStream_t st) {
    if (H % B3_TH != 0 || W % B3_TW != 0 || B < 1) return hipErrorInvalidValue;
    const int tiles_x = W / B3_TW, tiles_per_frame = tiles_x * (H / B3_TH), ntiles = B * tiles_per_frame;
    const int nstreams = conv2_wgrad_streams();
    if (nstreams < 8) return hipErrorInvalidValue;
    float *part = static_cast<float *>(workspace), *dbpart = part + (size_t)nstreams * 4 * (WG_OG * 9 * 64);
    once_per_device((const void *)k_conv2_wgrad_b16, [&] {
        (void)hipFuncSetAttribute((const void *)k_conv2_wgrad_b16, hipFuncAttributeMaxDynamicSharedMemorySize, WG_LDS);
    });
    hipLaunchKernelGGL(k_conv2_wgrad_b16, dim3(nstreams * 4), dim3(256), WG_LDS, st, dz, a1, H, W, tiles_x, tiles_per_frame, ntiles, nstreams, part, dbpart);
    hipLaunchKernelGGL(k_conv2_wgrad_finish, dim3(cdiv(128 * 9 * 64, 256)), dim3(256), 0, st, part, dbpart, nstreams, dw, db);
    return hipGetLastError();
}

__global__ void k_split_conv2_weights(const float *__restrict__ w, unsigned short *__restrict__ w2s_) {
    const int t = blockIdx.x * blockDim.x + threadIdx.x;
    if (t >= 9 * 64 * 128) return;
    const int c = t % 64, o = (t / 64) % 128, tap = t / (64 * 128);
    const float v = w[((size_t)o * 64 + c) * 9 + tap];
    __bf16 *w2s = reinterpret_cast<__bf16 *>(w2s_);
    __bf16 h, m, l;
    split3_bf16(v, h, m, l);
    const int ks2 = tap * 2 + (c >> 5), c32 = c & 31;
    w2s[((size_t)(ks2 * 3 + 0) * 128 + o) * 32 + c32] = h;
    w2s[((size_t)(ks2 * 3 + 1) * 128 + o) * 32 + c32] = m;
    w2s[((size_t)(ks2 * 3 + 2) * 128 + o) * 32 + c32] = l;
}

size_t conv2_train_workspace_bytes() { return (size_t)18 * 3 * 128 * 32 * sizeof(unsigned short); }

hipError_t launch_conv2_train_forward(const float *a1, const float *weight, const float *bias, int B, int H, int W, float *z2, void *workspace,
                                      hipStream_t st) {
    if (H % B3_TH != 0 || W % B3_TW != 0 || B < 1) return hipErrorInvalidValue;
    unsigned short *w2s = static_cast<unsigned short *>(workspace);
    hipLaunchKernelGGL(k_split_conv2_weights, dim3(cdiv(9 * 64 * 128, 256)), dim3(256), 0, st, weight, w2s);
    const int tiles_x = W / B3_TW, tiles_per_frame = tiles_x * (H / B3_TH), ntiles = B * tiles_per_frame;
    constexpr int lds = C2F_LDS;
    const int wgs_per_cu = device_cached_int((const void *)k_conv2_fwd_b16, [] {
        (void)hipFuncSetAttribute((const void *)k_conv2_fwd_b16, hipFuncAttributeMaxDynamicSharedMemorySize, lds);
        int n = 0;
        if (hipOccupancyMaxActiveBlocksPerMultiprocessor(&n, (const void *)k_conv2_fwd_b16, 256, lds) != hipSuccess || n < 1) n = 2;
        return n;
    });
    int nwg = device_num_cu() * wgs_per_cu;
    if (nwg > ntiles) nwg = ntiles;
    hipLaunchKernelGGL(k_conv2_fwd_b16, dim3(nwg), dim3(256), lds, st, a1, H, W, w2s, bias, z2, tiles_x, tiles_per_frame, ntiles);
    return hipGetLastError();
}

struct EncoderKnobs {
    int stagger, wgs_per_cu, shape;
    bool skip;
    EncoderKnobs() {
        const char *sv = getenv("SMK_ENC_STAGGER"), *ov = getenv("SMK_ENC_WGS_PER_CU"), *sh = getenv("SMK_ENC_SHAPE");
        const char *sk = getenv("SMK_ENC_SKIP");
        stagger = sv ? atoi(sv) : 1;
        wgs_per_cu = ov && atoi(ov) > 0 ? atoi(ov) : 0;
        shape = sh && atoi(sh) == 32 ? 32 : 16;
        skip = !(sk && atoi(sk) == 0);
    }
};
static const EncoderKnobs &enc_knobs() {
    static const EncoderKnobs k;
    return k;
}

constexpr int SCAN_ROWS = 4;
constexpr int SCAN_BR = 2 * SCAN_ROWS + 2;
constexpr int SCAN_FW = 256 / 4 + 2;
constexpr int ENC_FRAME_FEATS = 128 * 1024;

template <int PS, bool TOKENS, bool VEC>
__global__ __launch_bounds__(256) void k_encoder_tile_scan(const float *__restrict__ frames, int64_t fstride, int H, int W, int lg_tiles_x,
                                                           int bands_per_frame, const float *__restrict__ table,
                                                           float *__restrict__ features, unsigned long long *__restrict__ masks) {
    __shared__ unsigned int flag[SCAN_BR][SCAN_FW];
    __shared__ unsigned long long s_mask;
    const int tid = threadIdx.x;
    const int band = blockIdx.x, b = band / bands_per_frame, bi = band - b * bands_per_frame;
    const int tiles_x = 1 << lg_tiles_x, band_tiles = SCAN_ROWS * tiles_x;
    for (int i = tid; i < SCAN_BR * SCAN_FW; i += 256) (&flag[0][0])[i] = 0;
    __syncthreads();
    const int W4 = W >> 2, row0 = bi * (SCAN_ROWS * B3_TH) - 4;
    const unsigned int *src = reinterpret_cast<const unsigned int *>(frames) + (size_t)b * fstride;
    for (int i = tid; i < SCAN_BR * 4 * W4; i += 256) {
        const int rr = i / W4, c4 = i - rr * W4, row = row0 + rr;
        if (row < 0 || row >= H) continue;
        const unsigned int *p = src + (size_t)row * W + 4 * c4;
        unsigned int any;
        if (VEC) {
            const uint4 v = *reinterpret_cast<const uint4 *>(p);
            any = v.x | v.y | v.z | v.w;
        } else {
            any = p[0] | p[1] | p[2] | p[3];
        }
        if (any) flag[rr >> 2][c4 + 1] = 1;
    }
    __syncthreads();
    if (tid < 64) {
        unsigned int any = 0;
        if (tid < band_tiles) {
            const int tyl = tid >> lg_tiles_x, tx = tid & (tiles_x - 1);
#pragma unroll
            for (int br = 0; br < 4; ++br)
#pragma unroll
                for (int bc = 0; bc < 6; ++bc) any |= flag[2 * tyl + br][4 * tx + bc];
        }
        const unsigned long long m = __ballot(any != 0);
        if (tid == 0) {
            s_mask = m;
            masks[band] = m;
        }
    }
    __syncthreads();
    const unsigned long long m = s_mask;
    constexpr int CR = B3_TH / PS, CC = B3_TW / PS;
    float *out = features + (size_t)b * ENC_FRAME_FEATS;
    const int ty0 = bi * SCAN_ROWS;
    if (TOKENS) {
        constexpr int ROWV = CC * 32, UPT = CR * ROWV;
        for (int i = tid; i < band_tiles * UPT; i += 256) {
            const int tl = i / UPT, u = i - tl * UPT;
            if ((m >> tl) & 1) continue;
            const int ty = ty0 + (tl >> lg_tiles_x), tx = tl & (tiles_x - 1);
            const int a = u / ROWV, q = u - a * ROWV;
            const size_t off = (size_t)((ty * CR + a) * 32 + tx * CC) * 128 + q * 4;
            *reinterpret_cast<float4 *>(out + off) = *reinterpret_cast<const float4 *>(table + off);
        }
    } else {
        constexpr int VW = CC < 4 ? CC : 4, VPR = CC / VW, UPT = 128 * CR * VPR;
        for (int i = tid; i < band_tiles * UPT; i += 256) {
            const int tl = i / UPT, u = i - tl * UPT;
            if ((m >> tl) & 1) continue;
            const int ty = ty0 + (tl >> lg_tiles_x), tx = tl & (tiles_x - 1);
            const int v = u % VPR, a = (u / VPR) % CR, o = u / (VPR * CR);
            const size_t off = (size_t)o * 1024 + (ty * CR + a) * 32 + tx * CC + v * VW;
            if (VW == 2) *reinterpret_cast<float2 *>(out + off) = *reinterpret_cast<const float2 *>(table + off);
            else *reinterpret_cast<float4 *>(out + off) = *reinterpret_cast<const float4 *>(table + off);
        }
    }
}

constexpr int PACK_BANDS = 4;
__global__ __launch_bounds__(64 * PACK_BANDS) void k_encoder_tile_scan_pack(const unsigned long long *__restrict__ masks, int nbands,
                                                                            int lg_band_tiles, int *__restrict__ list,
                                                                            int *__restrict__ count) {
    __shared__ int part[PACK_BANDS];
    const int tid = threadIdx.x, lane = tid & 63, wave = tid >> 6;
    const int first = blockIdx.x * PACK_BANDS, band = first + wave;
    int c = 0;
    for (int j = tid; j < first; j += 64 * PACK_BANDS) c += __popcll(masks[j]);
#pragma unroll
    for (int d = 32; d >= 1; d >>= 1) c += __shfl_xor(c, d);
    if (lane == 0) part[wave] = c;
    __syncthreads();
    int before = 0;
#pragma unroll
    for (int w = 0; w < PACK_BANDS; ++w) before += part[w];
    if (band >= nbands) return;
    for (int w = 0; w < wave; ++w) before += __popcll(masks[first + w]);
    const unsigned long long m = masks[band];
    if ((m >> lane) & 1) list[before + __popcll(m & ((1ull << lane) - 1))] = (band << lg_band_tiles) + lane;
    if (band == nbands - 1 && lane == 0) *count = before + __popcll(m);
}

void EncoderSkip::release() {
    for (auto &f : table)
        for (auto &h : f)
            for (float *&t : h) {
                if (t) (void)hipFree(t);
                t = nullptr;
            }
    if (ws) (void)hipFree(ws);
    for (void *p : retired) (void)hipFree(p);
    retired.clear();
    ws = nullptr;
    ws_tiles = 0;
    last_count = nullptr;
}

hipError_t encoder_skip_stats(EncoderSkip &sk, int64_t *tiles_total, int64_t *tiles_run, hipStream_t st) {
    std::lock_guard<std::mutex> lk(sk.mu);
    hipError_t err = hipStreamSynchronize(st);
    if (err != hipSuccess) return err;
    int n = 0;
    if (sk.last_count && (err = hipMemcpy(&n, sk.last_count, sizeof(int), hipMemcpyDeviceToHost)) != hipSuccess) return err;
    *tiles_total = sk.last_total;
    *tiles_run = sk.last_count ? n : sk.last_total;
    return hipSuccess;
}

struct SkipPlan {
    const int *list = nullptr, *count = nullptr;
};

template <int FORM, bool TOKENS, class ZeroLaunch>
static hipError_t skip_prepare(EncoderSkip *sk, const float *frames, int64_t fstride, int B, int H, int W, float *features, int lg_tx,
                               int ntiles, int nwg, hipStream_t st, ZeroLaunch zero_launch, SkipPlan &plan) {
    if (!sk) return hipSuccess;
    std::lock_guard<std::mutex> lk(sk->mu);
    sk->last_total = ntiles;
    sk->last_count = nullptr;
    if (!enc_knobs().skip || ntiles <= nwg || (reinterpret_cast<uintptr_t>(features) & 15)) return hipSuccess;
    hipStreamCaptureStatus cs = hipStreamCaptureStatusNone;
    if (hipStreamIsCapturing(st, &cs) != hipSuccess) {
        (void)hipGetLastError();
        return hipSuccess;
    }
    const bool capturing = cs != hipStreamCaptureStatusNone;
    hipError_t err;
    float *&tab = sk->table[FORM][H == 64 ? 0 : H == 128 ? 1 : 2][TOKENS ? 1 : 0];
    if (!tab) {
        if (capturing) return hipSuccess;
        float *p = nullptr;
        if ((err = hipMalloc((void **)&p, ((size_t)ENC_FRAME_FEATS + (size_t)H * W) * sizeof(float))) != hipSuccess) return err;
        err = hipMemsetAsync(p + ENC_FRAME_FEATS, 0, (size_t)H * W * sizeof(float), st);
        if (err == hipSuccess) err = zero_launch(p + ENC_FRAME_FEATS, p);
        if (err != hipSuccess) {
            (void)hipFree(p);
            return err;
        }
        tab = p;
    }
    if (sk->ws_tiles < (size_t)ntiles) {
        if (capturing) return hipSuccess;
        int *p = nullptr;
        if ((err = hipMalloc((void **)&p, (4 + (size_t)ntiles / 8 + (size_t)ntiles) * sizeof(int))) != hipSuccess) return err;
        if (sk->ws) sk->retired.push_back(sk->ws);
        sk->ws = p;
        sk->ws_tiles = ntiles;
    }
    int *count = sk->ws, *list = sk->ws + 4 + sk->ws_tiles / 8;
    unsigned long long *masks = reinterpret_cast<unsigned long long *>(sk->ws + 4);
    const int bands_per_frame = H / B3_TH / SCAN_ROWS, nbands = B * bands_per_frame;
    const bool vec = (reinterpret_cast<uintptr_t>(frames) & 15) == 0 && (fstride & 3) == 0;
    dim3 grid(nbands), block(256);
#define SMK_SCAN_LAUNCH(PS_, VEC_)                                                                                                  \
    hipLaunchKernelGGL((k_encoder_tile_scan<PS_, TOKENS, VEC_>), grid, block, 0, st, frames, fstride, H, W, lg_tx, bands_per_frame, \
                       (const float *)tab, features, masks)
    switch (H / 32) {
        case 2: if (vec) SMK_SCAN_LAUNCH(2, true); else SMK_SCAN_LAUNCH(2, false); break;
        case 4: if (vec) SMK_SCAN_LAUNCH(4, true); else SMK_SCAN_LAUNCH(4, false); break;
        case 8: if (vec) SMK_SCAN_LAUNCH(8, true); else SMK_SCAN_LAUNCH(8, false); break;
        default: return hipErrorInvalidValue;
    }
#undef SMK_SCAN_LAUNCH
    if ((err = hipGetLastError()) != hipSuccess) return err;
    hipLaunchKernelGGL(k_encoder_tile_scan_pack, dim3((nbands + PACK_BANDS - 1) / PACK_BANDS), dim3(64 * PACK_BANDS), 0, st,
                       (const unsigned long long *)masks, nbands, lg_tx + 2, list, count);
    if ((err = hipGetLastError()) != hipSuccess) return err;
    plan.list = list;
    plan.count = count;
    sk->last_count = count;
    return hipSuccess;
}

template <bool TOKENS>
static hipError_t launch_b16_t(const float *frames, int64_t fstride, int B, int H, int W, const EncoderDev &e, float *features,
                               hipStream_t st, EncoderSkip *skip) {
    const int PS = H / 32;
    const int tiles_x = W / B3_TW, tiles_per_frame = tiles_x * (H / B3_TH), ntiles = B * tiles_per_frame;
    int lg_tx = 0, lg_tpf = 0;
    while ((1 << lg_tx) < tiles_x) ++lg_tx;
    while ((1 << lg_tpf) < tiles_per_frame) ++lg_tpf;
    if ((1 << lg_tx) != tiles_x || (1 << lg_tpf) != tiles_per_frame || (PS != 2 && PS != 4 && PS != 8)) return hipErrorInvalidValue;
    const int stagger = enc_knobs().stagger;
    const int num_cu = device_num_cu();
    const int wgs_per_cu = device_cached_int((const void *)k_encoder_b16<8, TOKENS>, [] {
        (void)hipFuncSetAttribute((const void *)k_encoder_b16<8, TOKENS>, hipFuncAttributeMaxDynamicSharedMemorySize, S16_LDS);
        (void)hipFuncSetAttribute((const void *)k_encoder_b16<4, TOKENS>, hipFuncAttributeMaxDynamicSharedMemorySize, S16_LDS);
        (void)hipFuncSetAttribute((const void *)k_encoder_b16<2, TOKENS>, hipFuncAttributeMaxDynamicSharedMemorySize, S16_LDS);
        int n = 0;
        if (hipOccupancyMaxActiveBlocksPerMultiprocessor(&n, (const void *)k_encoder_b16<8, TOKENS>, 256, S16_LDS) != hipSuccess || n < 1) n = 2;
        return enc_knobs().wgs_per_cu ? enc_knobs().wgs_per_cu : n;
    });
    auto run = [&](const float *fr, int64_t fs, int nt, float *out, const int *list, const int *count) -> hipError_t {
        int nwg = num_cu * wgs_per_cu;
        if (nwg > nt) nwg = nt;
        dim3 grid(nwg), block(256);
        switch (PS) {
            case 2: hipLaunchKernelGGL((k_encoder_b16<2, TOKENS>), grid, block, S16_LDS, st, fr, fs, H, W, e, out, lg_tx, lg_tpf, nt, stagger, list, count); break;
            case 4: hipLaunchKernelGGL((k_encoder_b16<4, TOKENS>), grid, block, S16_LDS, st, fr, fs, H, W, e, out, lg_tx, lg_tpf, nt, stagger, list, count); break;
            default: hipLaunchKernelGGL((k_encoder_b16<8, TOKENS>), grid, block, S16_LDS, st, fr, fs, H, W, e, out, lg_tx, lg_tpf, nt, stagger, list, count); break;
        }
        return hipGetLastError();
    };
    SkipPlan plan;
    hipError_t err = skip_prepare<0, TOKENS>(
        skip, frames, fstride, B, H, W, features, lg_tx, ntiles, num_cu * wgs_per_cu, st,
        [&](const float *zero_frame, float *table) { return run(zero_frame, (int64_t)H * W, tiles_per_frame, table, nullptr, nullptr); },
        plan);
    if (err != hipSuccess) return err;
    return run(frames, fstride, ntiles, features, plan.list, plan.count);
}

hipError_t launch_encoder_b16(const float *frames, int64_t fstride, int B, int H, int W, const EncoderDev &e, float *features,
                              bool tokens, hipStream_t st, EncoderSkip *skip) {
    return tokens ? launch_b16_t<true>(frames, fstride, B, H, W, e, features, st, skip)
                  : launch_b16_t<false>(frames, fstride, B, H, W, e, features, st, skip);
}

template <bool X3, bool TOKENS>
static hipError_t launch_bf16_t(const float *frames, int64_t fstride, int B, int H, int W, const EncoderDev &e,
                                float *features, hipStream_t st, EncoderSkip *skip) {
    const int PS = H / 32;
    const int tiles_x = W / B3_TW, tiles_per_frame = tiles_x * (H / B3_TH), ntiles = tiles_per_frame * B;
    int lg_tx = 0, lg_tpf = 0;
    while ((1 << lg_tx) < tiles_x) ++lg_tx;
    while ((1 << lg_tpf) < tiles_per_frame) ++lg_tpf;
    if ((1 << lg_tx) != tiles_x || (1 << lg_tpf) != tiles_per_frame || (PS != 2 && PS != 4 && PS != 8)) return hipErrorInvalidValue;
    const int stagger = enc_knobs().stagger;
    constexpr size_t lds_bytes = b3_lds_total<X3>();
    const int num_cu = device_num_cu();
    const int wgs_per_cu = device_cached_int((const void *)k_encoder_bf16<X3, 8, TOKENS>, [] {
        constexpr size_t lb = b3_lds_total<X3>();
        (void)hipFuncSetAttribute((const void *)k_encoder_bf16<X3, 8, TOKENS>, hipFuncAttributeMaxDynamicSharedMemorySize, (int)lb);
        (void)hipFuncSetAttribute((const void *)k_encoder_bf16<X3, 4, TOKENS>, hipFuncAttributeMaxDynamicSharedMemorySize, (int)lb);
        (void)hipFuncSetAttribute((const void *)k_encoder_bf16<X3, 2, TOKENS>, hipFuncAttributeMaxDynamicSharedMemorySize, (int)lb);
        int n = 0;
        if (hipOccupancyMaxActiveBlocksPerMultiprocessor(&n, (const void *)k_encoder_bf16<X3, 8, TOKENS>, 256, lb) != hipSuccess || n < 1) n = 2;
        return enc_knobs().wgs_per_cu ? enc_knobs().wgs_per_cu : n;
    });
    auto run = [&](const float *fr, int64_t fs, int nt, float *out, const int *list, const int *count) -> hipError_t {
        int nwg = num_cu * wgs_per_cu;
        if (nwg > nt) nwg = nt;
        dim3 grid(nwg), block(256);
        switch (PS) {
            case 2: hipLaunchKernelGGL((k_encoder_bf16<X3, 2, TOKENS>), grid, block, lds_bytes, st, fr, fs, H, W, e, out, lg_tx, lg_tpf, nt, stagger, list, count); break;
            case 4: hipLaunchKernelGGL((k_encoder_bf16<X3, 4, TOKENS>), grid, block, lds_bytes, st, fr, fs, H, W, e, out, lg_tx, lg_tpf, nt, stagger, list, count); break;
            default: hipLaunchKernelGGL((k_encoder_bf16<X3, 8, TOKENS>), grid, block, lds_bytes, st, fr, fs, H, W, e, out, lg_tx, lg_tpf, nt, stagger, list, count); break;
        }
        return hipGetLastError();
    };
    SkipPlan plan;
    hipError_t err = skip_prepare<X3 ? 0 : 1, TOKENS>(
        skip, frames, fstride, B, H, W, features, lg_tx, ntiles, num_cu * wgs_per_cu, st,
        [&](const float *zero_frame, float *table) { return run(zero_frame, (int64_t)H * W, tiles_per_frame, table, nullptr, nullptr); },
        plan);
    if (err != hipSuccess) return err;
    return run(frames, fstride, ntiles, features, plan.list, plan.count);
}

hipError_t launch_encoder_bf16(const float *frames, int64_t fstride, int B, int H, int W, const EncoderDev &e,
                               float *features, bool x3, bool tokens, hipStream_t st, EncoderSkip *skip) {
    const int shape = enc_knobs().shape;
    if (x3 && shape == 16) return launch_encoder_b16(frames, fstride, B, H, W, e, features, tokens, st, skip);
    if (x3) return tokens ? launch_bf16_t<true, true>(frames, fstride, B, H, W, e, features, st, skip)
                          : launch_bf16_t<true, false>(frames, fstride, B, H, W, e, features, st, skip);
    return tokens ? launch_bf16_t<false, true>(frames, fstride, B, H, W, e, features, st, skip)
                  : launch_bf16_t<false, false>(frames, fstride, B, H, W, e, features, st, skip);
}

typedef int i32x16 __attribute__((ext_vector_type(16)));
typedef int i32x4 __attribute__((ext_vector_type(4)));

constexpr int I8_A1_PITCH = 80;
constexpr int I8_A1_ROW = B3_AW * I8_A1_PITCH + 32;
constexpr int I8_A1_BYTES = (B3_TH + 2) * I8_A1_ROW;
constexpr int I8_LDS_BYTES = B3_XS_BYTES + 2 * I8_A1_BYTES + 2 * B3_W1_BYTES + B3_ST_BYTES + 64;

template <int PS, bool TOKENS>
__global__ __launch_bounds__(256, 2) void k_encoder_i8(const float *__restrict__ frames, int64_t fstride, int H, int W,
                                                    EncoderDev e, float *__restrict__ features, int lg_tiles_x,
                                                    int lg_tiles_per_frame, int ntiles,
                                                    const int *__restrict__ list, const int *__restrict__ count) {
    extern __shared__ __attribute__((aligned(16))) unsigned char smem[];
    float *xs = reinterpret_cast<float *>(smem);
    unsigned char *a1h = smem + B3_XS_BYTES, *a1l = a1h + I8_A1_BYTES;
    unsigned char *w1s = a1l + I8_A1_BYTES;
    float *st1 = reinterpret_cast<float *>(w1s + 2 * B3_W1_BYTES);
    float *wmx = st1 + 128;
    const int tid = threadIdx.x, lane = tid & 63, r = lane & 31, hi = lane >> 5;
    const int wave = __builtin_amdgcn_readfirstlane(tid >> 6);

    if (tid < 128) st1[tid] = tid < 64 ? e.s1[tid] : e.t1[tid - 64];
    {
        const uint4 *src = reinterpret_cast<const uint4 *>(e.w1p);
        for (int c = tid; c < 2 * 64 * 8; c += 256) {
            const int row = c >> 3, u = c & 7;
            *reinterpret_cast<uint4 *>(w1s + row * B3_W1_PITCH + u * 16) = src[c];
        }
    }
    const int o = wave * 32 + r;
    const float t2 = e.t2[o];
    const float scale_o = e.sw2[o] * e.s2[o];
    const int corr_h = e.wsum[o], corr_l = e.wsum[128 + o];
    const int lane_b = (o * 2 + hi) * 16;
    const __amdgpu_buffer_rsrc_t wrsrc =
        __builtin_amdgcn_make_buffer_rsrc(const_cast<signed char *>(e.w2i), 0, 18 * 2 * 4096, 0x00020000);
    typedef unsigned int u32x4 __attribute__((ext_vector_type(4)));
    auto load_b = [&](int kn, int part) -> i32x4 {
        const u32x4 v = __builtin_amdgcn_raw_buffer_load_b128(wrsrc, lane_b, (kn * 2 + part) * 4096, 0);
        return __builtin_bit_cast(i32x4, v);
    };
    constexpr int RING = 3;
    i32x4 bqh[RING], bql[RING];
#pragma unroll
    for (int k = 0; k < RING - 1; ++k) {
        bqh[k] = load_b(k, 0);
        bql[k] = load_b(k, 1);
    }
    const int lane_off = (r >> 4) * 4 * I8_A1_ROW + (r & 15) * I8_A1_PITCH + 16 * hi;

    auto x_fetch = [&](int t, int k) -> float {
        if (k >= B3_XH * B3_XW) return 0.f;
        const int bb = t >> lg_tiles_per_frame, rem = t & ((1 << lg_tiles_per_frame) - 1);
        const int rr0 = (rem >> lg_tiles_x) * B3_TH, cc0 = (rem & ((1 << lg_tiles_x) - 1)) * B3_TW;
        const int row = k / B3_XW, col = k - row * B3_XW;
        const int ii = rr0 - 4 + row, jj = cc0 - 4 + col;
        const bool ok = row < B3_XH - 1 && col < B3_XW - 1 && ii >= 0 && ii < H && jj >= 0 && jj < W;
        return ok ? frames[(size_t)bb * fstride + (size_t)ii * W + jj] : 0.f;
    };
    int k = blockIdx.x;
    const int nrun = tiles_to_run(list, count, ntiles);
    if (nrun == ntiles) list = nullptr;
    int t = k < nrun ? tile_at(list, k) : 0;
    if (k < nrun) {
        xs[tid] = x_fetch(t, tid);
        if (tid + 256 < B3_XH * B3_XW) xs[tid + 256] = x_fetch(t, tid + 256);
    }
    __syncthreads();

    for (; k < nrun; k += gridDim.x) {
        const int b = t >> lg_tiles_per_frame, rem = t & ((1 << lg_tiles_per_frame) - 1);
        const int r0 = (rem >> lg_tiles_x) * B3_TH, c0 = (rem & ((1 << lg_tiles_x) - 1)) * B3_TW;

        __builtin_amdgcn_s_setprio(0);
        float yv[3][16];
        int aoffs[2];
        bool valids[2];
        float vmax = 0.f;
        auto x_frags = [&](int pb, bf16x8 (&xh)[4], bf16x8 (&xl)[4], int &aoff, bool &valid, bool &inimg) {
            const int pix = pb * 32 + r;
            valid = pix < B3_APIX;
            const int pc = valid ? pix : B3_APIX - 1;
            const int ar = pc / B3_AW, ac = pc - ar * B3_AW;
            const int ii = r0 - 1 + ar, jj = c0 - 1 + ac;
            inimg = valid && ii >= 0 && ii < H && jj >= 0 && jj < W;
            aoff = ar * I8_A1_ROW + ac * I8_A1_PITCH;
            const float *xp = xs + (ar + hi) * B3_XW + ac;
#pragma unroll
            for (int s = 0; s < 4; ++s)
#pragma unroll
                for (int j = 0; j < 8; ++j) {
                    __bf16 vh, vl;
                    split_bf16(xp[s * 2 * B3_XW + j], vh, vl);
                    xh[s][j] = vh; xl[s][j] = vl;
                }
        };
        bool inimgs[2];
        auto bn1 = [&](const f32x16 &acc, int cb, bool inimg, float (&y)[16]) {
            float umax = 0.f;
#pragma unroll
            for (int q = 0; q < 4; ++q) {
                const int ch0 = cb * 32 + 8 * q + 4 * hi;
                const float4 sc = *reinterpret_cast<const float4 *>(st1 + ch0);
                const float4 sh = *reinterpret_cast<const float4 *>(st1 + 64 + ch0);
                const float scv[4] = {sc.x, sc.y, sc.z, sc.w}, shv[4] = {sh.x, sh.y, sh.z, sh.w};
#pragma unroll
                for (int i = 0; i < 4; ++i) {
                    const float v = bn_relu(acc[4 * q + i], scv[i], shv[i]);
                    y[4 * q + i] = v;
                    umax = fmaxf(umax, v);
                }
            }
            vmax = fmaxf(vmax, inimg ? umax : 0.f);
        };
        {
            bf16x8 xh[4], xl[4];
            bool inimg;
            x_frags(wave, xh, xl, aoffs[0], valids[0], inimg);
            inimgs[0] = inimg;
            f32x16 acc0, acc1;
#pragma unroll
            for (int g = 0; g < 16; ++g) { acc0[g] = 0.f; acc1[g] = 0.f; }
            const unsigned char *wrow = w1s + r * B3_W1_PITCH + 8 * hi * 2;
#pragma unroll
            for (int s = 0; s < 4; ++s) {
                const bf16x8 a0h = *reinterpret_cast<const bf16x8 *>(wrow + s * 32);
                const bf16x8 a1hh = *reinterpret_cast<const bf16x8 *>(wrow + 32 * B3_W1_PITCH + s * 32);
                const bf16x8 a0l = *reinterpret_cast<const bf16x8 *>(wrow + B3_W1_BYTES + s * 32);
                const bf16x8 a1l_ = *reinterpret_cast<const bf16x8 *>(wrow + B3_W1_BYTES + 32 * B3_W1_PITCH + s * 32);
                mma3<true>(acc0, a0h, a0l, xh[s], xl[s]);
                mma3<true>(acc1, a1hh, a1l_, xh[s], xl[s]);
            }
            bn1(acc0, 0, inimg, yv[0]);
            bn1(acc1, 1, inimg, yv[1]);
        }
        const int cbs = wave & 1;
        {
            bf16x8 xh[4], xl[4];
            bool inimg;
            x_frags(4 + (wave >> 1), xh, xl, aoffs[1], valids[1], inimg);
            inimgs[1] = inimg;
            f32x16 acc;
#pragma unroll
            for (int g = 0; g < 16; ++g) acc[g] = 0.f;
            const unsigned char *wrow = w1s + (cbs * 32 + r) * B3_W1_PITCH + 8 * hi * 2;
#pragma unroll
            for (int s = 0; s < 4; ++s) {
                const bf16x8 ah = *reinterpret_cast<const bf16x8 *>(wrow + s * 32);
                const bf16x8 al = *reinterpret_cast<const bf16x8 *>(wrow + B3_W1_BYTES + s * 32);
                mma3<true>(acc, ah, al, xh[s], xl[s]);
            }
            bn1(acc, cbs, inimg, yv[2]);
        }
#pragma unroll
        for (int off = 32; off > 0; off >>= 1) vmax = fmaxf(vmax, __shfl_xor(vmax, off));
        if (lane == 0) wmx[wave] = vmax;
        __syncthreads();
        const float tmax = fmaxf(fmaxf(wmx[0], wmx[1]), fmaxf(wmx[2], wmx[3]));
        const float invn = tmax > 0.f ? 65024.0f / (tmax * 65535.0f) : 0.f;
        const float s_tile = tmax > 0.f ? tmax / 65024.0f : 0.f;
        constexpr float OFFN = 128.0f / 65535.0f;
        auto quant_store = [&](const float (&y)[16], int cb, int aoff, bool valid, bool inimg) {
            if (!valid) return;
#pragma unroll
            for (int q = 0; q < 4; ++q) {
                const int ch0 = cb * 32 + 8 * q + 4 * hi;
                const unsigned int d0 = __builtin_bit_cast(unsigned int, __builtin_amdgcn_cvt_pknorm_u16(
                    fmaf(y[4 * q + 0], invn, OFFN), fmaf(y[4 * q + 1], invn, OFFN)));
                const unsigned int d1 = __builtin_bit_cast(unsigned int, __builtin_amdgcn_cvt_pknorm_u16(
                    fmaf(y[4 * q + 2], invn, OFFN), fmaf(y[4 * q + 3], invn, OFFN)));
                unsigned int ph = __builtin_amdgcn_perm(d1, d0, 0x07050301) ^ 0x80808080u;
                unsigned int pl = __builtin_amdgcn_perm(d1, d0, 0x06040200) ^ 0x80808080u;
                ph = inimg ? ph : 0x80808080u;
                pl = inimg ? pl : 0u;
                *reinterpret_cast<unsigned int *>(a1h + aoff + ch0) = ph;
                *reinterpret_cast<unsigned int *>(a1l + aoff + ch0) = pl;
            }
        };
        quant_store(yv[0], 0, aoffs[0], valids[0], inimgs[0]);
        quant_store(yv[1], 1, aoffs[0], valids[0], inimgs[0]);
        quant_store(yv[2], cbs, aoffs[1], valids[1], inimgs[1]);
        __syncthreads();
        __builtin_amdgcn_s_setprio(1);

        const int kn = k + gridDim.x;
        const int tn = kn < nrun ? tile_at(list, kn) : 0;
        float xr0 = 0.f, xr1 = 0.f;
        if (kn < nrun) {
            xr0 = x_fetch(tn, tid);
            xr1 = x_fetch(tn, tid + 256);
        }

        i32x16 hh[4], mid[4];
#pragma unroll
        for (int mi = 0; mi < 4; ++mi)
#pragma unroll
            for (int g = 0; g < 16; ++g) { hh[mi][g] = corr_h; mid[mi][g] = corr_l; }
        auto load_a = [&](int k, int pair, i32x4 (&ah)[2], i32x4 (&al)[2]) {
            const int tap = k >> 1, half = k & 1, ki = tap / 3, kj = tap - 3 * ki;
            const int abase = lane_off + ki * I8_A1_ROW + kj * I8_A1_PITCH + half * 32 + pair * 2 * I8_A1_ROW;
#pragma unroll
            for (int m = 0; m < 2; ++m) {
                ah[m] = *reinterpret_cast<const i32x4 *>(a1h + abase + m * I8_A1_ROW);
                al[m] = *reinterpret_cast<const i32x4 *>(a1l + abase + m * I8_A1_ROW);
            }
        };
        i32x4 ahA[2], alA[2], ahB[2], alB[2];
        load_a(0, 0, ahA, alA);
#pragma unroll 1
        for (int k0 = 0; k0 < 18; k0 += 6) {
#pragma unroll
            for (int u = 0; u < 6; ++u) {
                const int k = k0 + u;
                {
                    int kn = k + RING - 1;
                    kn = kn >= 18 ? kn - 18 : kn;
                    kn = __builtin_amdgcn_readfirstlane(kn);
                    bqh[(u + RING - 1) % RING] = load_b(kn, 0);
                    bql[(u + RING - 1) % RING] = load_b(kn, 1);
                }
                const i32x4 bh = bqh[u % RING], bl = bql[u % RING];
                load_a(k, 1, ahB, alB);
#pragma unroll
                for (int m = 0; m < 2; ++m) {
                    mid[m] = __builtin_amdgcn_mfma_i32_32x32x32_i8(alA[m], bh, mid[m], 0, 0, 0);
                    mid[m] = __builtin_amdgcn_mfma_i32_32x32x32_i8(ahA[m], bl, mid[m], 0, 0, 0);
                    hh[m] = __builtin_amdgcn_mfma_i32_32x32x32_i8(ahA[m], bh, hh[m], 0, 0, 0);
                }
#pragma unroll
                for (int i = 0; i < 6; ++i) {
                    __builtin_amdgcn_sched_group_barrier(0x008, 1, 0);
                    if (i < 4) __builtin_amdgcn_sched_group_barrier(0x100, 1, 0);
                    else __builtin_amdgcn_sched_group_barrier(0x020, 1, 0);
                }
                __builtin_amdgcn_sched_barrier(0);
                if (k + 1 < 18) load_a(k + 1, 0, ahA, alA);
#pragma unroll
                for (int m = 0; m < 2; ++m) {
                    mid[2 + m] = __builtin_amdgcn_mfma_i32_32x32x32_i8(alB[m], bh, mid[2 + m], 0, 0, 0);
                    mid[2 + m] = __builtin_amdgcn_mfma_i32_32x32x32_i8(ahB[m], bl, mid[2 + m], 0, 0, 0);
                    hh[2 + m] = __builtin_amdgcn_mfma_i32_32x32x32_i8(ahB[m], bh, hh[2 + m], 0, 0, 0);
                }
#pragma unroll
                for (int i = 0; i < 6; ++i) {
                    __builtin_amdgcn_sched_group_barrier(0x008, 1, 0);
                    if (i < 4) __builtin_amdgcn_sched_group_barrier(0x100, 1, 0);
                }
                __builtin_amdgcn_sched_barrier(0);
            }
        }

        const float sc = s_tile * scale_o * 256.0f;
        auto val = [&](int mi, int g) -> float {
            const float v = fmaf((float)hh[mi][g], 256.0f, (float)mid[mi][g]);
            const float y = fmaf(v, sc, t2);
            return y > 0.f ? y : 0.f;
        };
        auto out_index = [&](int pi, int pj) -> size_t {
            return TOKENS ? ((size_t)b * 1024 + pi * 32 + pj) * 128 + o : ((size_t)b * 128 + o) * 1024 + pi * 32 + pj;
        };
        if (PS == 2) {
#pragma unroll
            for (int mp = 0; mp < 2; ++mp)
#pragma unroll
                for (int qr = 0; qr < 2; ++qr)
#pragma unroll
                    for (int qc = 0; qc < 2; ++qc)
#pragma unroll
                        for (int cg = 0; cg < 2; ++cg) {
                            float sum = 0.f;
#pragma unroll
                            for (int mi = 2 * mp; mi < 2 * mp + 2; ++mi)
#pragma unroll
                                for (int i = 2 * cg; i < 2 * cg + 2; ++i) sum += val(mi, 4 * (2 * qr + qc) + i);
                            features[out_index((r0 + 2 * mp + 4 * qr) / 2, (c0 + 8 * qc + 4 * hi + 2 * cg) / 2)] = sum * 0.25f;
                        }
        } else if (PS == 4) {
#pragma unroll
            for (int qr = 0; qr < 2; ++qr)
#pragma unroll
                for (int qc = 0; qc < 2; ++qc) {
                    float sum = 0.f;
#pragma unroll
                    for (int mi = 0; mi < 4; ++mi)
#pragma unroll
                        for (int i = 0; i < 4; ++i) sum += val(mi, 4 * (2 * qr + qc) + i);
                    features[out_index((r0 + 4 * qr) / 4, (c0 + 8 * qc + 4 * hi) / 4)] = sum * (1.0f / 16);
                }
        } else {
            float cell[2];
#pragma unroll
            for (int qc = 0; qc < 2; ++qc) {
                float sum = 0.f;
#pragma unroll
                for (int mi = 0; mi < 4; ++mi)
#pragma unroll
                    for (int qr = 0; qr < 2; ++qr)
#pragma unroll
                        for (int i = 0; i < 4; ++i) sum += val(mi, 4 * (2 * qr + qc) + i);
                cell[qc] = sum;
            }
            const float other0 = __shfl_xor(cell[0], 32), other1 = __shfl_xor(cell[1], 32);
            const float total = hi == 0 ? cell[0] + other0 : cell[1] + other1;
            features[out_index(r0 / 8, c0 / 8 + hi)] = total * (1.0f / 64);
        }

        xs[tid] = xr0;
        if (tid + 256 < B3_XH * B3_XW) xs[tid + 256] = xr1;
        __syncthreads();
        t = tn;
    }
}

template <bool TOKENS>
static hipError_t launch_i8_t(const float *frames, int64_t fstride, int B, int H, int W, const EncoderDev &e, float *features,
                              hipStream_t st, EncoderSkip *skip) {
    const int PS = H / 32;
    const int tiles_x = W / B3_TW, tiles_per_frame = tiles_x * (H / B3_TH), ntiles = tiles_per_frame * B;
    int lg_tx = 0, lg_tpf = 0;
    while ((1 << lg_tx) < tiles_x) ++lg_tx;
    while ((1 << lg_tpf) < tiles_per_frame) ++lg_tpf;
    if ((1 << lg_tx) != tiles_x || (1 << lg_tpf) != tiles_per_frame || (PS != 2 && PS != 4 && PS != 8)) return hipErrorInvalidValue;
    constexpr size_t lds_bytes = I8_LDS_BYTES;
    const int num_cu = device_num_cu();
    const int wgs_per_cu = device_cached_int((const void *)k_encoder_i8<8, TOKENS>, [] {
        int n = 0;
        if (hipOccupancyMaxActiveBlocksPerMultiprocessor(&n, (const void *)k_encoder_i8<8, TOKENS>, 256, I8_LDS_BYTES) != hipSuccess || n < 1) n = 2;
        return enc_knobs().wgs_per_cu ? enc_knobs().wgs_per_cu : n;
    });
    auto run = [&](const float *fr, int64_t fs, int nt, float *out, const int *list, const int *count) -> hipError_t {
        int nwg = num_cu * wgs_per_cu;
        if (nwg > nt) nwg = nt;
        dim3 grid(nwg), block(256);
        switch (PS) {
            case 2: hipLaunchKernelGGL((k_encoder_i8<2, TOKENS>), grid, block, lds_bytes, st, fr, fs, H, W, e, out, lg_tx, lg_tpf, nt, list, count); break;
            case 4: hipLaunchKernelGGL((k_encoder_i8<4, TOKENS>), grid, block, lds_bytes, st, fr, fs, H, W, e, out, lg_tx, lg_tpf, nt, list, count); break;
            default: hipLaunchKernelGGL((k_encoder_i8<8, TOKENS>), grid, block, lds_bytes, st, fr, fs, H, W, e, out, lg_tx, lg_tpf, nt, list, count); break;
        }
        return hipGetLastError();
    };
    SkipPlan plan;
    hipError_t err = skip_prepare<2, TOKENS>(
        skip, frames, fstride, B, H, W, features, lg_tx, ntiles, num_cu * wgs_per_cu, st,
        [&](const float *zero_frame, float *table) { return run(zero_frame, (int64_t)H * W, tiles_per_frame, table, nullptr, nullptr); },
        plan);
    if (err != hipSuccess) return err;
    return run(frames, fstride, ntiles, features, plan.list, plan.count);
}

hipError_t launch_encoder_i8(const float *frames, int64_t fstride, int B, int H, int W, const EncoderDev &e, float *features,
                             bool tokens, hipStream_t st, EncoderSkip *skip) {
    return tokens ? launch_i8_t<true>(frames, fstride, B, H, W, e, features, st, skip)
                  : launch_i8_t<false>(frames, fstride, B, H, W, e, features, st, skip);
}

}
```

Before: 216,900.

## Fuse skip-list compaction and zero-tile fill into encoder kernels

```diff
diff --git a/smokephysai_amd/csrc/encoder.h b/smokephysai_amd/csrc/encoder.h
--- a/smokephysai_amd/csrc/encoder.h
+++ b/smokephysai_amd/csrc/encoder.h
@@ -23,7 +23,7 @@
     std::mutex mu;
     float *table[3][3][2] = {};
     int *ws = nullptr;
-    size_t ws_tiles = 0;
+    size_t ws_bands = 0;
     std::vector<void *> retired;
     int64_t last_total = 0;
     const int *last_count = nullptr;
diff --git a/smokephysai_amd/csrc/encoder.hip b/smokephysai_amd/csrc/encoder.hip
--- a/smokephysai_amd/csrc/encoder.hip
+++ b/smokephysai_amd/csrc/encoder.hip
@@ -302,18 +302,136 @@
 constexpr int B3_ST_BYTES = 2 * 64 * 4;
 template <bool X3> constexpr int b3_lds_total() { return b3_lds_bytes<X3>() + (X3 ? 2 : 1) * B3_W1_BYTES + B3_ST_BYTES; }
 
-__device__ __forceinline__ int tiles_to_run(const int *__restrict__ list, const int *__restrict__ count, int ntiles) {
-    return list ? __builtin_amdgcn_readfirstlane(*count) : ntiles;
-}
-__device__ __forceinline__ int tile_at(const int *__restrict__ list, int k) {
-    return list ? __builtin_amdgcn_readfirstlane(list[k]) : k;
-}
+struct SkipArgs {
+    const unsigned long long *masks = nullptr;
+    int *count = nullptr;
+    const float *table = nullptr;
+    int nbands = 0, lg_band_tiles = 0, bands_per_frame = 0;
+};
+constexpr int SCAN_ROWS = 4;
+constexpr int ENC_FRAME_FEATS = 128 * 1024;
+constexpr int SKIP_CHUNKS = 256, SKIP_SLATE = 16;
+struct SkipLds {
+    int cpre[SKIP_CHUNKS + 1];
+    int wsum[4];
+    int slate[SKIP_SLATE];
+};
+
+__device__ __forceinline__ int skip_lookup(const SkipLds &s, const SkipArgs &sa, int k) {
+    int c = 0;
+#pragma unroll
+    for (int step = SKIP_CHUNKS / 2; step >= 1; step >>= 1)
+        if (s.cpre[c + step] <= k) c += step;
+    int n = k - s.cpre[c];
+    int j = c * ((sa.nbands + SKIP_CHUNKS - 1) / SKIP_CHUNKS);
+    unsigned long long m = sa.masks[j];
+    for (int pc = __popcll(m); n >= pc; pc = __popcll(m)) {
+        n -= pc;
+        m = sa.masks[++j];
+    }
+    int pos = 0;
+#pragma unroll
+    for (int w = 32; w >= 1; w >>= 1) {
+        const int cnt = __popcll((m >> pos) & ((1ull << w) - 1));
+        if (n >= cnt) {
+            n -= cnt;
+            pos += w;
+        }
+    }
+    return (j << sa.lg_band_tiles) + pos;
+}
+
+__device__ __forceinline__ void skip_slate(SkipLds &s, const SkipArgs &sa, int r0, int nrun) {
+    const int i = threadIdx.x;
+    if (i < SKIP_SLATE) {
+        const long long k = (long long)blockIdx.x + (long long)(r0 + i) * gridDim.x;
+        if (k < nrun) s.slate[i] = skip_lookup(s, sa, (int)k);
+    }
+}
+
+__device__ __forceinline__ int tiles_to_run(SkipLds &s, const SkipArgs &sa, int ntiles) {
+    if (!sa.masks) return ntiles;
+    const int tid = threadIdx.x, lane = tid & 63, wave = tid >> 6;
+    const int cs = (sa.nbands + SKIP_CHUNKS - 1) / SKIP_CHUNKS;
+    int c = 0;
+    for (int j = tid * cs, je = min(j + cs, sa.nbands); j < je; ++j) c += __popcll(sa.masks[j]);
+    int inc = c;
+#pragma unroll
+    for (int d = 1; d < 64; d <<= 1) {
+        const int v = __shfl_up(inc, d);
+        if (lane >= d) inc += v;
+    }
+    if (lane == 63) s.wsum[wave] = inc;
+    __syncthreads();
+    int base = 0;
+    for (int w = 0; w < wave; ++w) base += s.wsum[w];
+    s.cpre[tid] = base + inc - c;
+    if (tid == SKIP_CHUNKS - 1) s.cpre[SKIP_CHUNKS] = base + inc;
+    __syncthreads();
+    const int nrun = __builtin_amdgcn_readfirstlane(s.cpre[SKIP_CHUNKS]);
+    if (blockIdx.x == 0 && tid == 0) *sa.count = nrun;
+    if (nrun != ntiles) {
+        skip_slate(s, sa, 0, nrun);
+        __syncthreads();
+    }
+    return nrun;
+}
+__device__ __forceinline__ int tile_at(SkipLds &s, const SkipArgs &sa, bool listed, int round, int k, int nrun) {
+    if (!listed) return k;
+    if (round > 0 && (round & (SKIP_SLATE - 1)) == 0) {
+        skip_slate(s, sa, round, nrun);
+        __syncthreads();
+    }
+    return __builtin_amdgcn_readfirstlane(s.slate[round & (SKIP_SLATE - 1)]);
+}
+
+template <int PS, bool TOKENS>
+__device__ __forceinline__ void skip_fill(const SkipArgs &sa, int lg_tiles_x, float *__restrict__ features) {
+    constexpr int CR = B3_TH / PS, CC = B3_TW / PS;
+    constexpr int VW = TOKENS ? 4 : (CC < 4 ? CC : 4), VPR = TOKENS ? 1 : CC / VW, ROWV = CC * 32;
+    constexpr int UPT = TOKENS ? CR * ROWV : 128 * CR * VPR;
+    constexpr int UNR = 4;
+    typedef float vec_t __attribute__((ext_vector_type(VW)));
+    const int tid = threadIdx.x, tiles_x = 1 << lg_tiles_x, band_tiles = 1 << sa.lg_band_tiles, total = band_tiles * UPT;
+    const unsigned long long full = band_tiles == 64 ? ~0ull : (1ull << band_tiles) - 1;
+    for (int band = blockIdx.x; band < sa.nbands; band += gridDim.x) {
+        const unsigned long long mv = sa.masks[band];
+        const unsigned long long m = ((unsigned long long)__builtin_amdgcn_readfirstlane((unsigned int)(mv >> 32)) << 32) |
+                                     (unsigned int)__builtin_amdgcn_readfirstlane((unsigned int)mv);
+        if (m == full) continue;
+        const int b = band / sa.bands_per_frame, ty0 = (band - b * sa.bands_per_frame) * SCAN_ROWS;
+        float *out = features + (size_t)b * ENC_FRAME_FEATS;
+        for (int i0 = tid; i0 < total; i0 += 256 * UNR) {
+            vec_t v[UNR];
+            int off[UNR];
+#pragma unroll
+            for (int j = 0; j < UNR; ++j) {
+                const int i = i0 + 256 * j, tl = i / UPT, u = i - tl * UPT;
+                off[j] = -1;
+                if (i >= total || ((m >> tl) & 1)) continue;
+                const int ty = ty0 + (tl >> lg_tiles_x), tx = tl & (tiles_x - 1);
+                if (TOKENS) {
+                    const int a = u / ROWV, q = u - a * ROWV;
+                    off[j] = ((ty * CR + a) * 32 + tx * CC) * 128 + q * 4;
+                } else {
+                    const int vv = u % VPR, a = (u / VPR) % CR, o = u / (VPR * CR);
+                    off[j] = o * 1024 + (ty * CR + a) * 32 + tx * CC + vv * VW;
+                }
+                v[j] = *reinterpret_cast<const vec_t *>(sa.table + off[j]);
+            }
+#pragma unroll
+            for (int j = 0; j < UNR; ++j)
+                if (off[j] >= 0) __builtin_nontemporal_store(v[j], reinterpret_cast<vec_t *>(out + off[j]));
+        }
+    }
+}
+__device__ __forceinline__ bool skip_fill_first() { return (blockIdx.x / 256) & 1; }
 
 template <bool X3, int PS, bool TOKENS>
 __global__ __launch_bounds__(256, 2) void k_encoder_bf16(const float *__restrict__ frames, int64_t fstride, int H, int W,
                                                       EncoderDev e, float *__restrict__ features, int lg_tiles_x,
                                                       int lg_tiles_per_frame, int ntiles, int stagger,
-                                                      const int *__restrict__ list, const int *__restrict__ count) {
+                                                      SkipArgs sa) {
     extern __shared__ __attribute__((aligned(16))) unsigned char smem[];
     float *xs = reinterpret_cast<float *>(smem);
     unsigned char *a1h = smem + B3_XS_BYTES, *a1l = a1h + B3_A1_BYTES;
@@ -360,10 +478,13 @@
         return ok ? frames[(size_t)bb * fstride + (size_t)ii * W + jj] : 0.f;
     };
     int k = blockIdx.x;
-    const int nrun = tiles_to_run(list, count, ntiles);
-    if (nrun == ntiles) list = nullptr;
-    int t = k < nrun ? tile_at(list, k) : 0;
-    if (stagger > 0 && ((blockIdx.x / 256) & 1))
+    __shared__ SkipLds skl;
+    const int nrun = tiles_to_run(skl, sa, ntiles);
+    const bool listed = nrun != ntiles;
+    int round = 0;
+    int t = k < nrun ? tile_at(skl, sa, listed, 0, k, nrun) : 0;
+    if (listed && skip_fill_first()) skip_fill<PS, TOKENS>(sa, lg_tiles_x, features);
+    else if (stagger > 0 && ((blockIdx.x / 256) & 1))
         for (int i = 0; i < stagger; ++i) __builtin_amdgcn_s_sleep(127);
     if (k < nrun) {
         xs[tid] = x_fetch(t, tid);
@@ -456,7 +577,8 @@
         __builtin_amdgcn_s_setprio(1);
 
         const int kn = k + gridDim.x;
-        const int tn = kn < nrun ? tile_at(list, kn) : 0;
+        ++round;
+        const int tn = kn < nrun ? tile_at(skl, sa, listed, round, kn, nrun) : 0;
         float xr0 = 0.f, xr1 = 0.f;
         if (kn < nrun) {
             xr0 = x_fetch(tn, tid);
@@ -566,6 +688,10 @@
         __syncthreads();
         t = tn;
     }
+    if (listed && !skip_fill_first()) {
+        __builtin_amdgcn_s_setprio(0);
+        skip_fill<PS, TOKENS>(sa, lg_tiles_x, features);
+    }
 }
 
 #ifndef S16_PRIO_CONV1
@@ -580,7 +706,7 @@
 __global__ __launch_bounds__(256, 2) void k_encoder_b16(const float *__restrict__ frames, int64_t fstride, int H, int W,
                                                      EncoderDev e, float *__restrict__ features, int lg_tiles_x,
                                                      int lg_tiles_per_frame, int ntiles, int stagger,
-                                                     const int *__restrict__ list, const int *__restrict__ count) {
+                                                     SkipArgs sa) {
     extern __shared__ __attribute__((aligned(16))) unsigned char smem[];
     unsigned int *xs = reinterpret_cast<unsigned int *>(smem);
     unsigned char *a1h = smem + B3_XS_BYTES, *a1l = a1h + S16_A1_BYTES;
@@ -633,10 +759,13 @@
         return (unsigned int)__builtin_bit_cast(unsigned short, vh) | ((unsigned int)__builtin_bit_cast(unsigned short, vl) << 16);
     };
     int k = blockIdx.x;
-    const int nrun = tiles_to_run(list, count, ntiles);
-    if (nrun == ntiles) list = nullptr;
-    int t = k < nrun ? tile_at(list, k) : 0;
-    if (stagger > 0 && ((blockIdx.x / 256) & 1))
+    __shared__ SkipLds skl;
+    const int nrun = tiles_to_run(skl, sa, ntiles);
+    const bool listed = nrun != ntiles;
+    int round = 0;
+    int t = k < nrun ? tile_at(skl, sa, listed, 0, k, nrun) : 0;
+    if (listed && skip_fill_first()) skip_fill<PS, TOKENS>(sa, lg_tiles_x, features);
+    else if (stagger > 0 && ((blockIdx.x / 256) & 1))
         for (int i = 0; i < stagger; ++i) __builtin_amdgcn_s_sleep(127);
     if (k < nrun) {
         xs[tid] = pack_split(x_fetch(t, tid));
@@ -741,7 +870,8 @@
         __builtin_amdgcn_s_setprio(S16_PRIO_KLOOP);
 
         const int kn = k + gridDim.x;
-        const int tn = kn < nrun ? tile_at(list, kn) : 0;
+        ++round;
+        const int tn = kn < nrun ? tile_at(skl, sa, listed, round, kn, nrun) : 0;
         float xr0 = 0.f, xr1 = 0.f;
         if (kn < nrun) {
             xr0 = x_fetch(tn, tid);
@@ -878,6 +1008,10 @@
         __syncthreads();
 #endif
         t = tn;
+    }
+    if (listed && !skip_fill_first()) {
+        __builtin_amdgcn_s_setprio(0);
+        skip_fill<PS, TOKENS>(sa, lg_tiles_x, features);
     }
 }
 
@@ -1633,17 +1767,13 @@
     return k;
 }
 
-constexpr int SCAN_ROWS = 4;
 constexpr int SCAN_BR = 2 * SCAN_ROWS + 2;
 constexpr int SCAN_FW = 256 / 4 + 2;
-constexpr int ENC_FRAME_FEATS = 128 * 1024;
-
-template <int PS, bool TOKENS, bool VEC>
+
+template <bool VEC>
 __global__ __launch_bounds__(256) void k_encoder_tile_scan(const float *__restrict__ frames, int64_t fstride, int H, int W, int lg_tiles_x,
-                                                           int bands_per_frame, const float *__restrict__ table,
-                                                           float *__restrict__ features, unsigned long long *__restrict__ masks) {
+                                                           int bands_per_frame, unsigned long long *__restrict__ masks) {
     __shared__ unsigned int flag[SCAN_BR][SCAN_FW];
-    __shared__ unsigned long long s_mask;
     const int tid = threadIdx.x;
     const int band = blockIdx.x, b = band / bands_per_frame, bi = band - b * bands_per_frame;
     const int tiles_x = 1 << lg_tiles_x, band_tiles = SCAN_ROWS * tiles_x;
@@ -1675,61 +1805,8 @@
                 for (int bc = 0; bc < 6; ++bc) any |= flag[2 * tyl + br][4 * tx + bc];
         }
         const unsigned long long m = __ballot(any != 0);
-        if (tid == 0) {
-            s_mask = m;
-            masks[band] = m;
-        }
-    }
-    __syncthreads();
-    const unsigned long long m = s_mask;
-    constexpr int CR = B3_TH / PS, CC = B3_TW / PS;
-    float *out = features + (size_t)b * ENC_FRAME_FEATS;
-    const int ty0 = bi * SCAN_ROWS;
-    if (TOKENS) {
-        constexpr int ROWV = CC * 32, UPT = CR * ROWV;
-        for (int i = tid; i < band_tiles * UPT; i += 256) {
-            const int tl = i / UPT, u = i - tl * UPT;
-            if ((m >> tl) & 1) continue;
-            const int ty = ty0 + (tl >> lg_tiles_x), tx = tl & (tiles_x - 1);
-            const int a = u / ROWV, q = u - a * ROWV;
-            const size_t off = (size_t)((ty * CR + a) * 32 + tx * CC) * 128 + q * 4;
-            *reinterpret_cast<float4 *>(out + off) = *reinterpret_cast<const float4 *>(table + off);
-        }
-    } else {
-        constexpr int VW = CC < 4 ? CC : 4, VPR = CC / VW, UPT = 128 * CR * VPR;
-        for (int i = tid; i < band_tiles * UPT; i += 256) {
-            const int tl = i / UPT, u = i - tl * UPT;
-            if ((m >> tl) & 1) continue;
-            const int ty = ty0 + (tl >> lg_tiles_x), tx = tl & (tiles_x - 1);
-            const int v = u % VPR, a = (u / VPR) % CR, o = u / (VPR * CR);
-            const size_t off = (size_t)o * 1024 + (ty * CR + a) * 32 + tx * CC + v * VW;
-            if (VW == 2) *reinterpret_cast<float2 *>(out + off) = *reinterpret_cast<const float2 *>(table + off);
-            else *reinterpret_cast<float4 *>(out + off) = *reinterpret_cast<const float4 *>(table + off);
-        }
-    }
-}
-
-constexpr int PACK_BANDS = 4;
-__global__ __launch_bounds__(64 * PACK_BANDS) void k_encoder_tile_scan_pack(const unsigned long long *__restrict__ masks, int nbands,
-                                                                            int lg_band_tiles, int *__restrict__ list,
-                                                                            int *__restrict__ count) {
-    __shared__ int part[PACK_BANDS];
-    const int tid = threadIdx.x, lane = tid & 63, wave = tid >> 6;
-    const int first = blockIdx.x * PACK_BANDS, band = first + wave;
-    int c = 0;
-    for (int j = tid; j < first; j += 64 * PACK_BANDS) c += __popcll(masks[j]);
-#pragma unroll
-    for (int d = 32; d >= 1; d >>= 1) c += __shfl_xor(c, d);
-    if (lane == 0) part[wave] = c;
-    __syncthreads();
-    int before = 0;
-#pragma unroll
-    for (int w = 0; w < PACK_BANDS; ++w) before += part[w];
-    if (band >= nbands) return;
-    for (int w = 0; w < wave; ++w) before += __popcll(masks[first + w]);
-    const unsigned long long m = masks[band];
-    if ((m >> lane) & 1) list[before + __popcll(m & ((1ull << lane) - 1))] = (band << lg_band_tiles) + lane;
-    if (band == nbands - 1 && lane == 0) *count = before + __popcll(m);
+        if (tid == 0) masks[band] = m;
+    }
 }
 
 void EncoderSkip::release() {
@@ -1743,7 +1820,7 @@
     for (void *p : retired) (void)hipFree(p);
     retired.clear();
     ws = nullptr;
-    ws_tiles = 0;
+    ws_bands = 0;
     last_count = nullptr;
 }
 
@@ -1758,13 +1835,9 @@
     return hipSuccess;
 }
 
-struct SkipPlan {
-    const int *list = nullptr, *count = nullptr;
-};
-
 template <int FORM, bool TOKENS, class ZeroLaunch>
 static hipError_t skip_prepare(EncoderSkip *sk, const float *frames, int64_t fstride, int B, int H, int W, float *features, int lg_tx,
-                               int ntiles, int nwg, hipStream_t st, ZeroLaunch zero_launch, SkipPlan &plan) {
+                               int ntiles, int nwg, hipStream_t st, ZeroLaunch zero_launch, SkipArgs &plan) {
     if (!sk) return hipSuccess;
     std::lock_guard<std::mutex> lk(sk->mu);
     sk->last_total = ntiles;
@@ -1790,35 +1863,29 @@
         }
         tab = p;
     }
-    if (sk->ws_tiles < (size_t)ntiles) {
+    const int bands_per_frame = H / B3_TH / SCAN_ROWS, nbands = B * bands_per_frame;
+    if (sk->ws_bands < (size_t)nbands) {
         if (capturing) return hipSuccess;
         int *p = nullptr;
-        if ((err = hipMalloc((void **)&p, (4 + (size_t)ntiles / 8 + (size_t)ntiles) * sizeof(int))) != hipSuccess) return err;
+        if ((err = hipMalloc((void **)&p, (4 + 2 * (size_t)nbands) * sizeof(int))) != hipSuccess) return err;
         if (sk->ws) sk->retired.push_back(sk->ws);
         sk->ws = p;
-        sk->ws_tiles = ntiles;
-    }
-    int *count = sk->ws, *list = sk->ws + 4 + sk->ws_tiles / 8;
+        sk->ws_bands = nbands;
+    }
+    int *count = sk->ws;
     unsigned long long *masks = reinterpret_cast<unsigned long long *>(sk->ws + 4);
-    const int bands_per_frame = H / B3_TH / SCAN_ROWS, nbands = B * bands_per_frame;
     const bool vec = (reinterpret_cast<uintptr_t>(frames) & 15) == 0 && (fstride & 3) == 0;
     dim3 grid(nbands), block(256);
-#define SMK_SCAN_LAUNCH(PS_, VEC_)                                                                                                  \
-    hipLaunchKernelGGL((k_encoder_tile_scan<PS_, TOKENS, VEC_>), grid, block, 0, st, frames, fstride, H, W, lg_tx, bands_per_frame, \
-                       (const float *)tab, features, masks)
-    switch (H / 32) {
-        case 2: if (vec) SMK_SCAN_LAUNCH(2, true); else SMK_SCAN_LAUNCH(2, false); break;
-        case 4: if (vec) SMK_SCAN_LAUNCH(4, true); else SMK_SCAN_LAUNCH(4, false); break;
-        case 8: if (vec) SMK_SCAN_LAUNCH(8, true); else SMK_SCAN_LAUNCH(8, false); break;
-        default: return hipErrorInvalidValue;
-    }
-#undef SMK_SCAN_LAUNCH
+    if (H != 64 && H != 128 && H != 256) return hipErrorInvalidValue;
+    if (vec) hipLaunchKernelGGL(k_encoder_tile_scan<true>, grid, block, 0, st, frames, fstride, H, W, lg_tx, bands_per_frame, masks);
+    else hipLaunchKernelGGL(k_encoder_tile_scan<false>, grid, block, 0, st, frames, fstride, H, W, lg_tx, bands_per_frame, masks);
     if ((err = hipGetLastError()) != hipSuccess) return err;
-    hipLaunchKernelGGL(k_encoder_tile_scan_pack, dim3((nbands + PACK_BANDS - 1) / PACK_BANDS), dim3(64 * PACK_BANDS), 0, st,
-                       (const unsigned long long *)masks, nbands, lg_tx + 2, list, count);
-    if ((err = hipGetLastError()) != hipSuccess) return err;
-    plan.list = list;
+    plan.masks = masks;
     plan.count = count;
+    plan.nbands = nbands;
+    plan.lg_band_tiles = lg_tx + 2;
+    plan.table = tab;
+    plan.bands_per_frame = bands_per_frame;
     sk->last_count = count;
     return hipSuccess;
 }
@@ -1842,24 +1909,24 @@
         if (hipOccupancyMaxActiveBlocksPerMultiprocessor(&n, (const void *)k_encoder_b16<8, TOKENS>, 256, S16_LDS) != hipSuccess || n < 1) n = 2;
         return enc_knobs().wgs_per_cu ? enc_knobs().wgs_per_cu : n;
     });
-    auto run = [&](const float *fr, int64_t fs, int nt, float *out, const int *list, const int *count) -> hipError_t {
+    auto run = [&](const float *fr, int64_t fs, int nt, float *out, const SkipArgs &sa) -> hipError_t {
         int nwg = num_cu * wgs_per_cu;
         if (nwg > nt) nwg = nt;
         dim3 grid(nwg), block(256);
         switch (PS) {
-            case 2: hipLaunchKernelGGL((k_encoder_b16<2, TOKENS>), grid, block, S16_LDS, st, fr, fs, H, W, e, out, lg_tx, lg_tpf, nt, stagger, list, count); break;
-            case 4: hipLaunchKernelGGL((k_encoder_b16<4, TOKENS>), grid, block, S16_LDS, st, fr, fs, H, W, e, out, lg_tx, lg_tpf, nt, stagger, list, count); break;
-            default: hipLaunchKernelGGL((k_encoder_b16<8, TOKENS>), grid, block, S16_LDS, st, fr, fs, H, W, e, out, lg_tx, lg_tpf, nt, stagger, list, count); break;
+            case 2: hipLaunchKernelGGL((k_encoder_b16<2, TOKENS>), grid, block, S16_LDS, st, fr, fs, H, W, e, out, lg_tx, lg_tpf, nt, stagger, sa); break;
+            case 4: hipLaunchKernelGGL((k_encoder_b16<4, TOKENS>), grid, block, S16_LDS, st, fr, fs, H, W, e, out, lg_tx, lg_tpf, nt, stagger, sa); break;
+            default: hipLaunchKernelGGL((k_encoder_b16<8, TOKENS>), grid, block, S16_LDS, st, fr, fs, H, W, e, out, lg_tx, lg_tpf, nt, stagger, sa); break;
         }
         return hipGetLastError();
     };
-    SkipPlan plan;
+    SkipArgs plan;
     hipError_t err = skip_prepare<0, TOKENS>(
         skip, frames, fstride, B, H, W, features, lg_tx, ntiles, num_cu * wgs_per_cu, st,
-        [&](const float *zero_frame, float *table) { return run(zero_frame, (int64_t)H * W, tiles_per_frame, table, nullptr, nullptr); },
+        [&](const float *zero_frame, float *table) { return run(zero_frame, (int64_t)H * W, tiles_per_frame, table, SkipArgs()); },
         plan);
     if (err != hipSuccess) return err;
-    return run(frames, fstride, ntiles, features, plan.list, plan.count);
+    return run(frames, fstride, ntiles, features, plan);
 }
 
 hipError_t launch_encoder_b16(const float *frames, int64_t fstride, int B, int H, int W, const EncoderDev &e, float *features,
@@ -1889,24 +1956,24 @@
         if (hipOccupancyMaxActiveBlocksPerMultiprocessor(&n, (const void *)k_encoder_bf16<X3, 8, TOKENS>, 256, lb) != hipSuccess || n < 1) n = 2;
         return enc_knobs().wgs_per_cu ? enc_knobs().wgs_per_cu : n;
     });
-    auto run = [&](const float *fr, int64_t fs, int nt, float *out, const int *list, const int *count) -> hipError_t {
+    auto run = [&](const float *fr, int64_t fs, int nt, float *out, const SkipArgs &sa) -> hipError_t {
         int nwg = num_cu * wgs_per_cu;
         if (nwg > nt) nwg = nt;
         dim3 grid(nwg), block(256);
         switch (PS) {
-            case 2: hipLaunchKernelGGL((k_encoder_bf16<X3, 2, TOKENS>), grid, block, lds_bytes, st, fr, fs, H, W, e, out, lg_tx, lg_tpf, nt, stagger, list, count); break;
-            case 4: hipLaunchKernelGGL((k_encoder_bf16<X3, 4, TOKENS>), grid, block, lds_bytes, st, fr, fs, H, W, e, out, lg_tx, lg_tpf, nt, stagger, list, count); break;
-            default: hipLaunchKernelGGL((k_encoder_bf16<X3, 8, TOKENS>), grid, block, lds_bytes, st, fr, fs, H, W, e, out, lg_tx, lg_tpf, nt, stagger, list, count); break;
+            case 2: hipLaunchKernelGGL((k_encoder_bf16<X3, 2, TOKENS>), grid, block, lds_bytes, st, fr, fs, H, W, e, out, lg_tx, lg_tpf, nt, stagger, sa); break;
+            case 4: hipLaunchKernelGGL((k_encoder_bf16<X3, 4, TOKENS>), grid, block, lds_bytes, st, fr, fs, H, W, e, out, lg_tx, lg_tpf, nt, stagger, sa); break;
+            default: hipLaunchKernelGGL((k_encoder_bf16<X3, 8, TOKENS>), grid, block, lds_bytes, st, fr, fs, H, W, e, out, lg_tx, lg_tpf, nt, stagger, sa); break;
         }
         return hipGetLastError();
     };
-    SkipPlan plan;
+    SkipArgs plan;
     hipError_t err = skip_prepare<X3 ? 0 : 1, TOKENS>(
         skip, frames, fstride, B, H, W, features, lg_tx, ntiles, num_cu * wgs_per_cu, st,
-        [&](const float *zero_frame, float *table) { return run(zero_frame, (int64_t)H * W, tiles_per_frame, table, nullptr, nullptr); },
+        [&](const float *zero_frame, float *table) { return run(zero_frame, (int64_t)H * W, tiles_per_frame, table, SkipArgs()); },
         plan);
     if (err != hipSuccess) return err;
-    return run(frames, fstride, ntiles, features, plan.list, plan.count);
+    return run(frames, fstride, ntiles, features, plan);
 }
 
 hipError_t launch_encoder_bf16(const float *frames, int64_t fstride, int B, int H, int W, const EncoderDev &e,
@@ -1931,7 +1998,7 @@
 __global__ __launch_bounds__(256, 2) void k_encoder_i8(const float *__restrict__ frames, int64_t fstride, int H, int W,
                                                     EncoderDev e, float *__restrict__ features, int lg_tiles_x,
                                                     int lg_tiles_per_frame, int ntiles,
-                                                    const int *__restrict__ list, const int *__restrict__ count) {
+                                                    SkipArgs sa) {
     extern __shared__ __attribute__((aligned(16))) unsigned char smem[];
     float *xs = reinterpret_cast<float *>(smem);
     unsigned char *a1h = smem + B3_XS_BYTES, *a1l = a1h + I8_A1_BYTES;
@@ -1980,9 +2047,12 @@
         return ok ? frames[(size_t)bb * fstride + (size_t)ii * W + jj] : 0.f;
     };
     int k = blockIdx.x;
-    const int nrun = tiles_to_run(list, count, ntiles);
-    if (nrun == ntiles) list = nullptr;
-    int t = k < nrun ? tile_at(list, k) : 0;
+    __shared__ SkipLds skl;
+    const int nrun = tiles_to_run(skl, sa, ntiles);
+    const bool listed = nrun != ntiles;
+    int round = 0;
+    int t = k < nrun ? tile_at(skl, sa, listed, 0, k, nrun) : 0;
+    if (listed && skip_fill_first()) skip_fill<PS, TOKENS>(sa, lg_tiles_x, features);
     if (k < nrun) {
         xs[tid] = x_fetch(t, tid);
         if (tid + 256 < B3_XH * B3_XW) xs[tid + 256] = x_fetch(t, tid + 256);
@@ -2105,7 +2175,8 @@
         __builtin_amdgcn_s_setprio(1);
 
         const int kn = k + gridDim.x;
-        const int tn = kn < nrun ? tile_at(list, kn) : 0;
+        ++round;
+        const int tn = kn < nrun ? tile_at(skl, sa, listed, round, kn, nrun) : 0;
         float xr0 = 0.f, xr1 = 0.f;
         if (kn < nrun) {
             xr0 = x_fetch(tn, tid);
@@ -2230,6 +2301,10 @@
         if (tid + 256 < B3_XH * B3_XW) xs[tid + 256] = xr1;
         __syncthreads();
         t = tn;
+    }
+    if (listed && !skip_fill_first()) {
+        __builtin_amdgcn_s_setprio(0);
+        skip_fill<PS, TOKENS>(sa, lg_tiles_x, features);
     }
 }
 
@@ -2249,24 +2324,24 @@
         if (hipOccupancyMaxActiveBlocksPerMultiprocessor(&n, (const void *)k_encoder_i8<8, TOKENS>, 256, I8_LDS_BYTES) != hipSuccess || n < 1) n = 2;
         return enc_knobs().wgs_per_cu ? enc_knobs().wgs_per_cu : n;
     });
-    auto run = [&](const float *fr, int64_t fs, int nt, float *out, const int *list, const int *count) -> hipError_t {
+    auto run = [&](const float *fr, int64_t fs, int nt, float *out, const SkipArgs &sa) -> hipError_t {
         int nwg = num_cu * wgs_per_cu;
         if (nwg > nt) nwg = nt;
         dim3 grid(nwg), block(256);
         switch (PS) {
-            case 2: hipLaunchKernelGGL((k_encoder_i8<2, TOKENS>), grid, block, lds_bytes, st, fr, fs, H, W, e, out, lg_tx, lg_tpf, nt, list, count); break;
-            case 4: hipLaunchKernelGGL((k_encoder_i8<4, TOKENS>), grid, block, lds_bytes, st, fr, fs, H, W, e, out, lg_tx, lg_tpf, nt, list, count); break;
-            default: hipLaunchKernelGGL((k_encoder_i8<8, TOKENS>), grid, block, lds_bytes, st, fr, fs, H, W, e, out, lg_tx, lg_tpf, nt, list, count); break;
+            case 2: hipLaunchKernelGGL((k_encoder_i8<2, TOKENS>), grid, block, lds_bytes, st, fr, fs, H, W, e, out, lg_tx, lg_tpf, nt, sa); break;
+            case 4: hipLaunchKernelGGL((k_encoder_i8<4, TOKENS>), grid, block, lds_bytes, st, fr, fs, H, W, e, out, lg_tx, lg_tpf, nt, sa); break;
+            default: hipLaunchKernelGGL((k_encoder_i8<8, TOKENS>), grid, block, lds_bytes, st, fr, fs, H, W, e, out, lg_tx, lg_tpf, nt, sa); break;
         }
         return hipGetLastError();
     };
-    SkipPlan plan;
+    SkipArgs plan;
     hipError_t err = skip_prepare<2, TOKENS>(
         skip, frames, fstride, B, H, W, features, lg_tx, ntiles, num_cu * wgs_per_cu, st,
-        [&](const float *zero_frame, float *table) { return run(zero_frame, (int64_t)H * W, tiles_per_frame, table, nullptr, nullptr); },
+        [&](const float *zero_frame, float *table) { return run(zero_frame, (int64_t)H * W, tiles_per_frame, table, SkipArgs()); },
         plan);
     if (err != hipSuccess) return err;
-    return run(frames, fstride, ntiles, features, plan.list, plan.count);
+    return run(frames, fstride, ntiles, features, plan);
 }
 
 hipError_t launch_encoder_i8(const float *frames, int64_t fstride, int B, int H, int W, const EncoderDev &e, float *features,
```

Result: faster. 222,200, median of 6 (+2.5%).
